# SilentView/EMCID

Measured on AMD Instinct MI355X. Metric: concept-edits/sec (1 000-concept batch, SD-v1.4), higher is better.
Workload: dtype f32 forward (2 x fp16 split MFMA, fp32 accumulate) + f64 solve

## Files before the change

### emcid_amd/csrc/clip_layers.hip

```cpp
#include "common.h"

#include <algorithm>

namespace emcid {

__global__ __launch_bounds__(256) void gather_rows16_kernel(const unsigned char* __restrict__ src, int64_t src_stride,
                                                             const int* __restrict__ idx, unsigned char* __restrict__ dst,
                                                             int64_t dst_stride, int row_bytes) {
    typedef unsigned int v4u __attribute__((ext_vector_type(4)));
    const int64_t r = blockIdx.x;
    const v4u* s = reinterpret_cast<const v4u*>(src + (int64_t)idx[r] * src_stride);
    v4u* d = reinterpret_cast<v4u*>(dst + r * dst_stride);
    for (int i = threadIdx.x; i < row_bytes / 16; i += 256) d[i] = s[i];
}

__global__ __launch_bounds__(256) void gather_f32_kernel(const float* __restrict__ src, const int* __restrict__ idx,
                                                          float* __restrict__ dst, int n) {
    const int i = blockIdx.x * 256 + threadIdx.x;
    if (i < n) dst[i] = src[idx[i]];
}

__device__ __forceinline__ unsigned long long fp_mix(unsigned long long x) {
    x ^= x >> 30; x *= 0xBF58476D1CE4E5B9ull; x ^= x >> 27; x *= 0x94D049BB133111EBull; x ^= x >> 31;
    return x;
// ... 37 lines not shown
        long long* e = table + 4 * b.slot[blockIdx.x];
        e[0] = (long long)reinterpret_cast<uintptr_t>(data); e[1] = bytes; e[2] = (long long)h; e[3] = 0;
    }
}

struct FpSkip { unsigned long long m[4]; };

__global__ __launch_bounds__(256) void fingerprint_check_kernel(const long long* table, long long first_slot, FpSkip skip, int* flag) {
    __shared__ unsigned long long lds[4];
    if ((skip.m[blockIdx.x >> 6] >> (blockIdx.x & 63)) & 1ull) return;
    const long long* e = table + 4 * (first_slot + blockIdx.x);
    const long long bytes = e[1];
    if (bytes <= 0) return;
    const unsigned long long h = fingerprint_of(reinterpret_cast<const unsigned char*>((uintptr_t)e[0]), bytes, lds);
    if (threadIdx.x == 0 && h != (unsigned long long)e[2]) atomicOr(flag, 1);
}

struct ClipWs {
    float* qkv;
    float* mid;
    uint32_t* ctx_p;
    float* ctx_s;
    uint32_t* z_p;
    float* z_s;
    float* f_scale;
    uint32_t* f_p;
    uint32_t* xq_p;
    float* xq_s;
    float* hs_q;
};

inline int64_t clip_ws_bytes(int64_t rows, int64_t h, int64_t d) {
    const int64_t r = round_up(rows, 64);
    return 4 * (r * 3 * h + r * h + r * h + r + r * h + r + 2 * r + r * d + r * h + r + r * h) + 16 * 16;
}

inline bool clip_ws_carve(void* base, int64_t bytes, int64_t rows, int64_t h, int64_t d, ClipWs& w) {
    if (base == nullptr || !aligned16(base) || bytes < clip_ws_bytes(rows, h, d)) return false;
    const int64_t r = round_up(rows, 64);
    char* p = (char*)base;
    auto take = [&](int64_t n4) { char* q = p; p += round_up(4 * n4, 16); return q; };
    w.qkv = (float*)take(r * 3 * h);
    w.mid = (float*)take(r * h);
    w.ctx_p = (uint32_t*)take(r * h);
    w.ctx_s = (float*)take(r);
    w.z_p = (uint32_t*)take(r * h);
    w.z_s = (float*)take(r);
    w.f_scale = (float*)take(2 * r);
    w.f_p = (uint32_t*)take(r * d);
    w.xq_p = (uint32_t*)take(r * h);
    w.xq_s = (float*)take(r);
    w.hs_q = (float*)take(r * h);
    return true;
}

}

using namespace emcid;

extern "C" {

int emcid_fingerprint_store(int64_t n, const void* const* data, const int64_t* bytes, const int64_t* slots, void* table,
                            int64_t table_slots, void* stream) {
    EMCID_CHECK_ARG(n >= 0 && table && (n == 0 || (data && bytes && slots)));
    for (int64_t i0 = 0; i0 < n; i0 += 32) {
        FpBatch b{};
        const int cnt = (int)std::min<int64_t>(32, n - i0);
        for (int i = 0; i < cnt; ++i) {
            EMCID_CHECK_ARG(data[i0 + i] && bytes[i0 + i] > 0 && bytes[i0 + i] % 16 == 0 && aligned16(data[i0 + i]) &&
                            slots[i0 + i] >= 0 && slots[i0 + i] < table_slots);
            b.data[i] = (const unsigned char*)data[i0 + i]; b.bytes[i] = bytes[i0 + i]; b.slot[i] = slots[i0 + i];
        }
        hipLaunchKernelGGL(fingerprint_store_kernel, dim3((unsigned)cnt), dim3(256), 0, (hipStream_t)stream, b, (long long*)table);
    }
    EMCID_CHECK_LAUNCH();
    return EMCID_OK;
}

int emcid_fingerprint_check(const void* table, int64_t table_slots, int64_t first_slot, int64_t n_slots, const uint64_t* skip_mask,
                            int* flag, void* stream) {
    EMCID_CHECK_ARG(table && flag && first_slot >= 0 && n_slots >= 0 && first_slot + n_slots <= table_slots && n_slots <= 256);
    if (n_slots == 0) return EMCID_OK;
    FpSkip skip{};
    if (skip_mask != nullptr)
        for (int w = 0; w < 4; ++w) skip.m[w] = skip_mask[w];
    hipLaunchKernelGGL(fingerprint_check_kernel, dim3((unsigned)n_slots), dim3(256), 0, (hipStream_t)stream, (const long long*)table,
                       (long long)first_slot, skip, flag);
    EMCID_CHECK_LAUNCH();
    return EMCID_OK;
}

int64_t emcid_clip_workspace_bytes(int64_t rows, int64_t h, int64_t d) { return clip_ws_bytes(rows, h, d); }

int emcid_clip_layer_head_sp16(const emcid_clip_layer_sp16* L, int64_t rows, int64_t h, int64_t d, int64_t heads, float attn_scale,
                               const int* anc, int64_t anc_ld, const int* depth, const int* rows_sel, int64_t n_sel,
                               const float* hs, const void* x_planes, const float* x_inv_scale, float* mid, void* f_planes,
                               float* f_scale, float* f_f32, void* workspace, int64_t workspace_bytes, void* stream) {
    EMCID_CHECK_ARG(L && rows > 0 && h > 0 && d > 0 && heads > 0 && h % heads == 0 && anc && depth && hs && x_planes && x_inv_scale);
    EMCID_CHECK_ARG(mid && f_planes && f_scale && n_sel > 0 && n_sel <= rows && (rows_sel != nullptr || n_sel == rows) && h % 32 == 0 && d % 32 == 0);
    ClipWs w;
    if (!clip_ws_carve(workspace, workspace_bytes, rows, h, d, w)) return fail(EMCID_ERR_BAD_ARG, __func__, "workspace too small or misaligned");
    hipStream_t st = (hipStream_t)stream;
    const int64_t D = h / heads;
    const float* q;
    int64_t ldq;
    const float* res;
    if (rows_sel == nullptr) {
        EMCID_TRY(emcid_linear_sp16_f32(x_planes, h, x_inv_scale, L->qkv_planes, h, L->qkv_inv_scale, L->qkv_bias, nullptr, 0, w.qkv,
                                        3 * h, nullptr, 0, nullptr, rows, 3 * h, h, 0, -1, stream));
        q = w.qkv, ldq = 3 * h, res = hs;
    } else {
        EMCID_TRY(emcid_linear_sp16_f32(x_planes, h, x_inv_scale, (const uint32_t*)L->qkv_planes + h * h, h, L->qkv_inv_scale + h,
                                        L->qkv_bias ? L->qkv_bias + h : nullptr, nullptr, 0, w.qkv + h, 3 * h, nullptr, 0, nullptr,
                                        rows, 2 * h, h, 0, -1, stream));
        {
            ScopedProf sp(KC_MISC, st);
            hipLaunchKernelGGL(gather_rows16_kernel, dim3((unsigned)n_sel), dim3(256), 0, st, (const unsigned char*)x_planes, 4 * h,
                               rows_sel, (unsigned char*)w.xq_p, 4 * h, (int)(4 * h));
            hipLaunchKernelGGL(gather_f32_kernel, dim3((unsigned)((n_sel + 255) / 256)), dim3(256), 0, st, x_inv_scale, rows_sel,
                               w.xq_s, (int)n_sel);
            hipLaunchKernelGGL(gather_rows16_kernel, dim3((unsigned)n_sel), dim3(256), 0, st, (const unsigned char*)hs, 4 * h,
                               rows_sel, (unsigned char*)w.hs_q, 4 * h, (int)(4 * h));
            EMCID_CHECK_LAUNCH();
        }
        EMCID_TRY(emcid_linear_sp16_f32(w.xq_p, h, w.xq_s, L->qkv_planes, h, L->qkv_inv_scale, L->qkv_bias, nullptr, 0, w.mid, h,
                                        nullptr, 0, nullptr, n_sel, h, h, 0, -1, stream));
        q = w.mid, ldq = h, res = w.hs_q;
    }
    EMCID_TRY(emcid_tree_attention_sp16(q, ldq, w.qkv + h, w.qkv + 2 * h, 3 * h, anc, anc_ld, depth, rows_sel, n_sel, heads, D,
                                        attn_scale, w.ctx_p, h, w.ctx_s, stream));
    EMCID_TRY(emcid_linear_sp16_f32(w.ctx_p, h, w.ctx_s, L->out_planes, h, L->out_inv_scale, L->out_bias, res, h, mid, h, nullptr,
                                    0, nullptr, n_sel, h, h, 0, -1, stream));
    EMCID_TRY(emcid_add_layernorm_sp16(mid, h, nullptr, 0, L->ln2_gamma, L->ln2_beta, L->ln2_eps, n_sel, h, nullptr, nullptr, w.z_p,
                                       h, w.z_s, L->fc1_bound, f_scale, stream));
    EMCID_TRY(emcid_linear_sp16_f32(w.z_p, h, w.z_s, L->fc1_planes, h, L->fc1_inv_scale, L->fc1_bias, nullptr, 0, f_f32, d,
                                    f_planes, d, f_scale, n_sel, d, h, L->act, -1, stream));
    return EMCID_OK;
}

int emcid_clip_layer_tail_sp16(const emcid_clip_layer_sp16* L, int64_t n, int64_t h, int64_t d, const void* f_planes,
                               const float* f_inv_scale, const float* mid, float* hs_out, const float* next_ln_gamma,
                               const float* next_ln_beta, float next_ln_eps, void* x_planes, float* x_inv_scale, void* stream) {
    EMCID_CHECK_ARG(L && n > 0 && h % 32 == 0 && d % 32 == 0 && f_planes && f_inv_scale && mid && hs_out);
    EMCID_TRY(emcid_linear_sp16_f32(f_planes, d, f_inv_scale, L->fc2_planes, d, L->fc2_inv_scale, L->fc2_bias, mid, h, hs_out, h,
                                    nullptr, 0, nullptr, n, h, d, 0, -1, stream));
    if (next_ln_gamma != nullptr) {
        EMCID_CHECK_ARG(next_ln_beta && x_planes && x_inv_scale);
        EMCID_TRY(emcid_add_layernorm_sp16(hs_out, h, nullptr, 0, next_ln_gamma, next_ln_beta, next_ln_eps, n, h, nullptr, nullptr,
                                           x_planes, h, x_inv_scale, nullptr, nullptr, stream));
    }
    return EMCID_OK;
}

int emcid_clip_edit_layer_tail_sp16(const emcid_clip_layer_sp16* L, int64_t n_rows, int64_t h, int64_t d, const float* f_f32,
                                    const void* f_planes, const float* f_inv_scale, const float* mid, const int64_t* lookup,
                                    const int64_t* seg, int64_t B, int64_t N, const float* zs_t, double edit_weight,
                                    int layers_left, double lam_ratio, const void* cov_factor_ws, int64_t n_layers,
                                    int64_t layer_index, int use_inverse, const float* W0, float* W, float* dW, float* K_out,
                                    float* Zc_out, void* k_planes, float* k_inv_scale, void* dual_ws, int64_t dual_ws_bytes,
                                    int* info_dev, void* linear_ws, int64_t linear_ws_bytes, float* hs_out,
                                    const float* next_ln_gamma, const float* next_ln_beta, float next_ln_eps, void* x_planes,
                                    float* x_inv_scale, void* stream) {
    EMCID_CHECK_ARG(L && n_rows > 0 && h % 32 == 0 && d % 32 == 0 && f_f32 && lookup && seg && B > 0 && N > 0 && zs_t);
    EMCID_CHECK_ARG(cov_factor_ws && W0 && W && K_out && Zc_out && dual_ws && info_dev && (hs_out == nullptr || (f_planes && f_inv_scale && mid)));
    EMCID_TRY(emcid_gather_mean_f32(f_f32, B, n_rows, d, 0, d, lookup, seg, N, K_out, d, stream));
    EMCID_CHECK_ARG((k_planes == nullptr) == (k_inv_scale == nullptr));
    if (k_planes != nullptr) {
        EMCID_TRY(emcid_split_rows_f16(K_out, d, N, d, k_planes, d, k_inv_scale, nullptr, stream));
        EMCID_TRY(emcid_linear_sp16_f32(k_planes, d, k_inv_scale, L->fc2_planes, d, L->fc2_inv_scale, L->fc2_bias, nullptr, 0, Zc_out, h,
                                        nullptr, 0, nullptr, N, h, d, 0, -1, stream));
    } else {
        EMCID_TRY(emcid_linear_ws_f32(K_out, d, W, d, L->fc2_bias, nullptr, 0, Zc_out, h, N, h, d, 0, -1, linear_ws, linear_ws_bytes, stream));
    }
    EMCID_TRY(emcid_edit_dual_apply_stage1_f64(K_out, Zc_out, zs_t, N, d, h, edit_weight, layers_left, lam_ratio, cov_factor_ws,
                                               n_layers, layer_index, 0, N, use_inverse, dual_ws, dual_ws_bytes, stream));
    EMCID_TRY(emcid_edit_dual_apply_stage2_f64(N, d, h, cov_factor_ws, n_layers, layer_index, use_inverse, 0, W0, W, dW, dual_ws,
                                               dual_ws_bytes, info_dev, stream));
    if (hs_out != nullptr) {
        EMCID_TRY(emcid_split_rows_f16(W, d, h, d, const_cast<void*>(L->fc2_planes), d, const_cast<float*>(L->fc2_inv_scale), nullptr,
                                       stream));
        EMCID_TRY(emcid_clip_layer_tail_sp16(L, n_rows, h, d, f_planes, f_inv_scale, mid, hs_out, next_ln_gamma, next_ln_beta,
                                             next_ln_eps, x_planes, x_inv_scale, stream));
    }
    return EMCID_OK;
}

int emcid_clip_layers_sp16(const emcid_clip_layer_sp16* layers, int64_t n_layers, int64_t rows, int64_t h, int64_t d, int64_t heads,
                           float attn_scale, const int* anc, int64_t anc_ld, const int* depth, float* hs, void* x_planes,
                           float* x_inv_scale, const float* next_ln_gamma, const float* next_ln_beta, float next_ln_eps,
                           void* workspace, int64_t workspace_bytes, void* stream) {
    EMCID_CHECK_ARG(layers && n_layers > 0 && hs && x_planes && x_inv_scale);
    ClipWs w;
    if (!clip_ws_carve(workspace, workspace_bytes, rows, h, d, w)) return fail(EMCID_ERR_BAD_ARG, __func__, "workspace too small or misaligned");
    for (int64_t i = 0; i < n_layers; ++i) {
        const emcid_clip_layer_sp16* L = layers + i;
        EMCID_TRY(emcid_clip_layer_head_sp16(L, rows, h, d, heads, attn_scale, anc, anc_ld, depth, nullptr, rows, hs, x_planes,
                                             x_inv_scale, w.mid, w.f_p, w.f_scale, nullptr, workspace, workspace_bytes, stream));
        const bool last = i + 1 == n_layers;
        const float* g = last ? next_ln_gamma : layers[i + 1].ln1_gamma;
        const float* b = last ? next_ln_beta : layers[i + 1].ln1_beta;
        const float eps = last ? next_ln_eps : layers[i + 1].ln1_eps;
        EMCID_TRY(emcid_clip_layer_tail_sp16(L, rows, h, d, w.f_p, w.f_scale + rows, w.mid, hs, g, b, eps, x_planes, x_inv_scale, stream));
    }
    return EMCID_OK;
}

}
```

### emcid_amd/csrc/edit_solve.hip

```cpp
#include "spd_solve.h"

namespace emcid {


__global__ __launch_bounds__(256) void prep_kr_kernel(const float* __restrict__ K, const float* __restrict__ Zc,
                                                       const float* __restrict__ zs_t, int N, int d, int h, double s,
                                                       double layers_left, double* __restrict__ Kt64, int Np, int dp,
                                                       double* __restrict__ Rt, int hp, double g = 1.0) {
    const int n = blockIdx.x;
    for (int j = threadIdx.x; j < dp; j += 256) {
        double v = 0.0;
        if (n < N && j < d) v = (double)K[(int64_t)n * d + j] * s * g;
        Kt64[(int64_t)n * dp + j] = v;
    }
    if (Rt) {
        for (int i = threadIdx.x; i < hp; i += 256) {
            double v = 0.0;
            if (n < N && i < h) {
                const float src = zs_t[(int64_t)n * h + i] - Zc[(int64_t)n * h + i];
                v = ((double)src * s) / layers_left * g;
            }
            Rt[(int64_t)n * hp + i] = v;
        }
    }
}

static void launch_prep_kr(const float* K, const float* Zc, const float* zs_t, int64_t N, int64_t d, int64_t h, double edit_weight,
                           int layers_left, double gain, double* Kt, int64_t Np, int64_t dp, double* R, int64_t hp, hipStream_t st) {
    ScopedProf sp(KC_PREP, st);
    hipLaunchKernelGGL(prep_kr_kernel, dim3((unsigned)Np), dim3(256), 0, st, K, Zc, zs_t, (int)N, (int)d, (int)h, sqrt(edit_weight / 0.5),
                       (double)layers_left, Kt, (int)Np, (int)dp, R, (int)hp, gain);
}

__global__ __launch_bounds__(256) void axpy_f32_kernel(float* __restrict__ W, const float* __restrict__ dW, int64_t n) {
    int64_t i = (int64_t)blockIdx.x * 256 + threadIdx.x;
    const int64_t stride = (int64_t)gridDim.x * 256;
    for (; i < n; i += stride) W[i] += dW[i];
}

__global__ __launch_bounds__(256) void apply_u_kernel(const double* __restrict__ U, const float* __restrict__ W0,
                                                       float* __restrict__ W, float* __restrict__ dW, int64_t n) {
    int64_t i = (int64_t)blockIdx.x * 256 + threadIdx.x;
    const int64_t stride = (int64_t)gridDim.x * 256;
    for (; i < n; i += stride) {
        const float f = (float)U[i];
        if (dW) dW[i] = f;
        if (W) W[i] = W0[i] + f;
    }
}

static int factor_and_solve(double* A, double* L, int64_t dp, int64_t lda, double* invw, int* info, double* B, double* Y,
                            int64_t rows, int64_t ldb, hipStream_t st) {
    return with_graph(make_key(GRAPH_FACTOR_SOLVE, {A, L, invw, info, B, Y}, {dp, lda, rows, ldb}), st, [&](hipStream_t s) {
        EMCID_TRY(cholesky_impl(A, L, dp, lda, invw, info, s));
        return cholesky_solve_impl(L, dp, lda, invw, B, Y, rows, ldb, s);
    });
}


struct CovPtrs { const float* c[32]; };
__global__ __launch_bounds__(256) void scale_cov_kernel(CovPtrs cov, int d, int dp, double lam, float cw, double* __restrict__ M,
                                                         int64_t s_mat) {
    const int l = blockIdx.y;
    const int i = blockIdx.x;
    const float* C = cov.c[l];
    double* row = M + l * s_mat + (int64_t)i * dp;
    for (int j = threadIdx.x; j <= i; j += 256) {
        double v;
        if (i < d) {
            const float c1 = C[(int64_t)i * d + j] * cw;
            v = lam * (double)(c1 / 0.5f);
        } else {
            v = (i == j) ? 1.0 : 0.0;
        }
        row[j] = v;
    }
}

static void assemble_dual_system(const double* P, const double* Q, int64_t dp, double* S, int Np, hipStream_t st,
                                 double* sk_work = nullptr) {
    ScopedProf sp(KC_ASSEMBLE, st);
    GemmShape g{P, dp, Q, dp, Np, Np, (int)dp, 1};
    if (Np >= 512 && sk_work && launch_gemm_f64_streamk2<true, true>(g, EpiAxpby{S, Np, 1.0, 0.0}, st, kStreamKWgs, sk_work, 1.0))
        return;
    hipLaunchKernelGGL(eye_f64_kernel, dim3((unsigned)Np), dim3(256), 0, st, S, Np);
    const int kt = (int)(dp / 16);
    g.ksplit = kt >= 64 ? 4 : kt >= 32 ? 2 : 1;
    launch_gemm_f64<true, true>(g, EpiAxpby{S, Np, 1.0, 1.0}, st, Np >= 512 ? 1 : 2);
}

__global__ __launch_bounds__(256) void transpose_f64_kernel(const double* __restrict__ src, int64_t lds_, double* __restrict__ dst,
                                                             int64_t ldd, int rows, int cols) {
    __shared__ double tile[32][33];
    const int bx = blockIdx.x * 32, by = blockIdx.y * 32;
    const int tx = threadIdx.x & 31, ty = threadIdx.x >> 5;
    for (int r = ty; r < 32; r += 8)
        tile[r][tx] = (by + r < rows && bx + tx < cols) ? src[(int64_t)(by + r) * lds_ + bx + tx] : 0.0;
    __syncthreads();
    for (int r = ty; r < 32; r += 8)
        if (bx + r < cols && by + tx < rows) dst[(int64_t)(bx + r) * ldd + by + tx] = tile[tx][r];
}

struct EditWorkspace {
    int64_t Np, dp, hp;
    int64_t off_A, off_L, off_inv, off_B, off_Y, off_R, total;
    EditWorkspace(int64_t N, int64_t d, int64_t h) {
        Np = round_up(N, NPAD);
        dp = round_up(d, NB);
        hp = round_up(h, 2);
        int64_t o = 0;
        off_A = o; o += dp * dp;
        off_L = o; o += dp * dp;
        off_inv = o; o += inv_doubles(dp);
        off_B = o; o += Np * dp;
        off_Y = o; o += Np * dp;
        off_R = o; o += Np * hp;
        total = o;
    }
};

int solve_schur_rhs(const double* R, int64_t hp, int64_t h, int64_t Np, const double* LS, const double* invS, const double* XT,
                    double* full_inv, double* RT, double* Y2, hipStream_t st) {
    hipLaunchKernelGGL(transpose_f64_kernel, dim3((unsigned)((hp + 31) / 32), (unsigned)(Np / 32)), dim3(256), 0, st, R, hp, RT, Np,
                       (int)Np, (int)hp);
    if (XT) {
        ScopedProf sp(KC_TRSM_DIAG, st);
        GemmShape f{RT, Np, XT, Np, (int)h, (int)Np, (int)Np, 0};
        f.tri = 1; f.pair = 1;
        launch_gemm_f64<true, false>(f, EpiAxpby{Y2, Np, 1.0, 0.0}, st);
        GemmShape b{Y2, Np, XT, Np, (int)h, (int)Np, (int)Np, 0};
        b.tri = 2; b.pair = 1;
        launch_gemm_f64<true, true>(b, EpiAxpby{RT, Np, 1.0, 0.0}, st);
    } else if (full_inv && Np <= 4096) {
        EMCID_TRY(build_full_inverse(LS, Np, Np, invS, full_inv, Y2, 1, 0, 0, st));
        ScopedProf sp(KC_TRSM_DIAG, st);
        GemmShape f{RT, Np, full_inv, Np, (int)h, (int)Np, (int)Np, 0};
        f.tri = 1; f.pair = 1;
        launch_gemm_f64<true, true>(f, EpiAxpby{Y2, Np, 1.0, 0.0}, st);
        GemmShape b{Y2, Np, full_inv, Np, (int)h, (int)Np, (int)Np, 0};
        b.tri = 2; b.pair = 1;
        launch_gemm_f64<true, false>(b, EpiAxpby{RT, Np, 1.0, 0.0}, st);
    } else {
        EMCID_TRY(cholesky_solve_impl(LS, Np, Np, invS, RT, Y2, h, Np, st));
    }
    return EMCID_OK;
}

}

using namespace emcid;

extern "C" {

int emcid_assemble_spd_f64(const float* C, int64_t ldc, const double* Kt64, int64_t Np, int64_t d, int64_t ldk, double lam,
                           float cw, double* A, int64_t lda, void* stream) {
    EMCID_CHECK_ARG(C && Kt64 && A && Np > 0 && d > 0);
    const int64_t dp = round_up(d, NB);
    EMCID_CHECK_ARG(lda >= dp && ldk >= dp && ldc >= d && (ldk % 2 == 0) && aligned16(Kt64));
    GemmShape p{Kt64, ldk, Kt64, ldk, (int)dp, (int)dp, (int)Np, 1};
    {
        ScopedProf sp(KC_ASSEMBLE, (hipStream_t)stream);
        launch_gemm_f64<false, false>(p, EpiAssemble{C, ldc, lam, cw, A, lda, (int)d}, (hipStream_t)stream);
    }
    EMCID_CHECK_LAUNCH();
    return EMCID_OK;
}

int emcid_delta_w_f64(const double* Rt, int64_t ldr, const double* Xt, int64_t ldx, int64_t Np, int64_t h, int64_t d,
                      const float* W0, float* W, int64_t ldw, float* dW, double* U, void* stream) {
    EMCID_CHECK_ARG(Rt && Xt && Np > 0 && h > 0 && d > 0 && ldr % 2 == 0 && ldx % 2 == 0 && aligned16(Rt) && aligned16(Xt));
    EMCID_CHECK_ARG((W == nullptr) || (W0 != nullptr));
    GemmShape p{Rt, ldr, Xt, ldx, (int)h, (int)d, (int)Np, 0};
    {
        ScopedProf sp(KC_DELTA_W, (hipStream_t)stream);
        launch_gemm_f64<false, false>(p, EpiDeltaW{W0, W, ldw, dW, d, U, d}, (hipStream_t)stream);
    }
    EMCID_CHECK_LAUNCH();
    return EMCID_OK;
}

int emcid_axpy_f32(float* W, const float* dW, int64_t n, void* stream) {
    EMCID_CHECK_ARG(W && dW && n > 0);
    int64_t blocks = (n + 255) / 256;
    if (blocks > 2048) blocks = 2048;
    hipLaunchKernelGGL(axpy_f32_kernel, dim3((unsigned)blocks), dim3(256), 0, (hipStream_t)stream, W, dW, n);
    EMCID_CHECK_LAUNCH();
    return EMCID_OK;
}

int64_t emcid_edit_workspace_bytes(int64_t N, int64_t d, int64_t h) {
    if (N <= 0 || d <= 0 || h <= 0) return 0;
    return EditWorkspace(N, d, h).total * (int64_t)sizeof(double);
}

static int edit_layer_impl(const float* K, const float* Zc, const float* zs_t, const float* C, int64_t N, int64_t d, int64_t h,
                           double lam, double edit_weight, int layers_left, int64_t n_lo, int64_t n_hi, const float* W0,
                           float* W, double* Xt_out, double* Rt_out, float* dW_out, double* U_out, void* workspace,
                           int64_t workspace_bytes, int* info_dev, void* stream) {
    EMCID_CHECK_ARG(K && Zc && zs_t && C && N > 0 && d > 0 && h > 0 && layers_left > 0 && workspace && info_dev);
    EMCID_CHECK_ARG(N < (1 << 24) && d <= 32768 && h <= 32768);
    EMCID_CHECK_ARG(0 <= n_lo && n_lo < n_hi && n_hi <= N);
    EMCID_CHECK_ARG((W == nullptr) || (W0 != nullptr));
    EMCID_CHECK_ARG(aligned16(workspace));
    EditWorkspace ws(N, d, h);
    EMCID_CHECK_WORKSPACE(workspace_bytes, ws.total * (int64_t)sizeof(double), " (see emcid_edit_workspace_bytes)");
    hipStream_t st = (hipStream_t)stream;
    double* base = (double*)workspace;
    double *A = base + ws.off_A, *L = base + ws.off_L, *inv = base + ws.off_inv;
    double *B = base + ws.off_B, *Y = base + ws.off_Y, *R = base + ws.off_R;
    const float cw = (float)(1.0 - edit_weight);
    const int64_t rows = n_hi - n_lo;

    launch_prep_kr(K, Zc, zs_t, N, d, h, edit_weight, layers_left, 1.0, B, ws.Np, ws.dp, R, ws.hp, st);
    EMCID_CHECK_LAUNCH();
    EMCID_TRY(emcid_assemble_spd_f64(C, d, B, ws.Np, d, ws.dp, lam, cw, A, ws.dp, stream));
    double* Bs = B + n_lo * ws.dp;
    EMCID_TRY(factor_and_solve(A, L, ws.dp, ws.dp, inv, info_dev, Bs, Y + n_lo * ws.dp, rows, ws.dp, st));
    if (W || dW_out || U_out)
        EMCID_TRY(emcid_delta_w_f64(R + n_lo * ws.hp, ws.hp, Bs, ws.dp, rows, h, d, W0, W, d, dW_out, U_out, stream));
    if (Xt_out)
        hipLaunchKernelGGL(copy2d_f64_kernel, dim3((unsigned)rows), dim3(256), 0, st, Bs, ws.dp, Xt_out, d, (int)rows, (int)d);
    if (Rt_out)
        hipLaunchKernelGGL(copy2d_f64_kernel, dim3((unsigned)rows), dim3(256), 0, st, R + n_lo * ws.hp, ws.hp, Rt_out, h,
                           (int)rows, (int)h);
    EMCID_CHECK_LAUNCH();
    return EMCID_OK;
}

int emcid_edit_layer_f64(const float* K, const float* Zc, const float* zs_t, const float* C, int64_t N, int64_t d, int64_t h,
                         double lam, double edit_weight, int layers_left, const float* W0, float* W, double* Xt_out,
                         double* Rt_out, float* dW_out, void* workspace, int64_t workspace_bytes, int* info_dev,
                         void* stream) {
    return edit_layer_impl(K, Zc, zs_t, C, N, d, h, lam, edit_weight, layers_left, 0, N, W0, W, Xt_out, Rt_out, dW_out,
                           nullptr, workspace, workspace_bytes, info_dev, stream);
}

int emcid_edit_layer_shard_f64(const float* K, const float* Zc, const float* zs_t, const float* C, int64_t N, int64_t d,
                               int64_t h, double lam, double edit_weight, int layers_left, int64_t n_lo, int64_t n_hi,
                               double* U_partial, double* Xt_out, double* Rt_out, void* workspace, int64_t workspace_bytes,
                               int* info_dev, void* stream) {
    EMCID_CHECK_ARG(U_partial != nullptr);
    return edit_layer_impl(K, Zc, zs_t, C, N, d, h, lam, edit_weight, layers_left, n_lo, n_hi, nullptr, nullptr, Xt_out,
                           Rt_out, nullptr, U_partial, workspace, workspace_bytes, info_dev, stream);
}

int emcid_apply_update_f32(const double* U, const float* W0, float* W, float* dW, int64_t n, void* stream) {
    EMCID_CHECK_ARG(U && n > 0 && (W || dW) && ((W == nullptr) || (W0 != nullptr)));
    int64_t blocks = (n + 255) / 256;
    if (blocks > 2048) blocks = 2048;
    hipLaunchKernelGGL(apply_u_kernel, dim3((unsigned)blocks), dim3(256), 0, (hipStream_t)stream, U, W0, W, dW, n);
    EMCID_CHECK_LAUNCH();
    return EMCID_OK;
}


int64_t emcid_cov_factor_workspace_bytes(int64_t n_layers, int64_t d) {
    if (n_layers <= 0 || d <= 0) return 0;
    return CovFactorLayout(n_layers, d).total * (int64_t)sizeof(double);
}

int emcid_factor_cov_f64(const float* const* C_host_list, int64_t n_layers, int64_t d, double lam, double edit_weight,
                         void* workspace, int64_t workspace_bytes, int* info_dev, void* stream) {
    EMCID_CHECK_ARG(C_host_list && n_layers > 0 && n_layers <= 32 && d > 0 && d <= 32768 && workspace && info_dev);
    EMCID_CHECK_ARG(aligned16(workspace));
    const CovFactorLayout cov(n_layers, d);
    EMCID_CHECK_WORKSPACE(workspace_bytes, cov.total * (int64_t)sizeof(double), " (see emcid_cov_factor_workspace_bytes)");
    const int64_t dp = cov.dp, s_mat = cov.s_mat, s_inv = cov.s_inv;
    double *Mb = cov.M(workspace, 0), *Lb = cov.L(workspace, 0), *Ib = cov.I(workspace, 0);
    CovPtrs cp;
    for (int i = 0; i < 32; ++i) cp.c[i] = i < n_layers ? C_host_list[i] : nullptr;
    for (int i = 0; i < n_layers; ++i) EMCID_CHECK_ARG(cp.c[i] != nullptr);
    const float cw = (float)(1.0 - edit_weight);
    hipStream_t st = (hipStream_t)stream;
    GraphKey key = make_key(GRAPH_FACTOR_COV, {Mb, info_dev}, {n_layers, d, 0, 0, 0});
    memcpy(&key.num[2], &lam, sizeof(double));
    memcpy(&key.num[3], &cw, sizeof(float));
    for (int i = 0; i < n_layers; ++i)
        if (i < 6) key.ptr[2 + i] = cp.c[i]; else key.num[4] = key.num[4] * 1000003 + (int64_t)(uintptr_t)cp.c[i];
    return with_graph(key, st, [&](hipStream_t s) {
        hipLaunchKernelGGL(scale_cov_kernel, dim3((unsigned)dp, (unsigned)n_layers), dim3(256), 0, s, cp, (int)d, (int)dp, lam, cw,
                           Mb, s_mat);
        return cholesky_serial(Mb, Lb, dp, dp, Ib, info_dev, s, (int)n_layers, s_mat, s_inv);
    });
}

int emcid_cov_inverse_f64(void* cov_factor_ws, int64_t n_layers, int64_t d, int64_t first_layer, int64_t count, void* stream) {
    EMCID_CHECK_ARG(cov_factor_ws && n_layers > 0 && n_layers <= 32 && d > 0 && d <= 32768 && aligned16(cov_factor_ws));
    EMCID_CHECK_ARG(0 <= first_layer && count > 0 && first_layer + count <= n_layers);
    const CovFactorLayout cov(n_layers, d);
    const int64_t dp = cov.dp;
    double* Mb = cov.M(cov_factor_ws, first_layer);
    const double *Lb = cov.L(cov_factor_ws, first_layer), *Ib = cov.I(cov_factor_ws, first_layer);
    double* Xb = cov.X(cov_factor_ws, first_layer);
    return with_graph(make_key(GRAPH_COV_INVERSE, {Mb, Lb, Ib, Xb}, {dp, count}), (hipStream_t)stream, [&](hipStream_t s) {
        return build_full_inverse(Lb, dp, dp, Ib, Xb, Mb, (int)count, cov.s_mat, cov.s_inv, s);
    });
}

__global__ __launch_bounds__(256) void cov_factor_rescale_kernel(const double* src, double* dst, int64_t off_L, int64_t off_I,
                                                                 int64_t off_X, int64_t s_mat, int64_t s_inv, int dp, int n_tri,
                                                                 double gain_L, double gain_inv, int with_inverse) {
    const int64_t layer = blockIdx.y;
    const int region = blockIdx.z;
    if (region == 1) {
        const double2* s = reinterpret_cast<const double2*>(src + off_I + layer * s_inv);
        double2* o = reinterpret_cast<double2*>(dst + off_I + layer * s_inv);
        for (int64_t i = (int64_t)blockIdx.x * 256 + threadIdx.x; i < s_inv / 2; i += (int64_t)gridDim.x * 256) {
            double2 v = s[i];
            v.x *= gain_inv;
            v.y *= gain_inv;
            o[i] = v;
        }
        return;
    }
    if (region == 2 && !with_inverse) return;
    const int t = blockIdx.x;
    if (t >= n_tri) return;
    int I = (int)((sqrtf(8.0f * (float)t + 1.0f) - 1.0f) * 0.5f);
    while ((I + 1) * (I + 2) / 2 <= t) ++I;
    while (I * (I + 1) / 2 > t) --I;
    const int J = t - I * (I + 1) / 2;
    const int64_t base = (region == 0 ? off_L : off_X) + layer * s_mat + (int64_t)I * NB * dp + (int64_t)J * NB;
    const double g = region == 0 ? gain_L : gain_inv;
    for (int e = threadIdx.x; e < NB * (NB / 2); e += 256) {
        const int r = e / (NB / 2), c2 = e % (NB / 2);
        const int64_t at = base + (int64_t)r * dp + 2 * c2;
        double2 v = *reinterpret_cast<const double2*>(src + at);
        v.x *= g;
        v.y *= g;
        *reinterpret_cast<double2*>(dst + at) = v;
    }
}

int emcid_cov_factor_rescale_f64(const void* src_ws, void* dst_ws, int64_t workspace_bytes, int64_t n_layers, int64_t d, double a,
                                 int with_inverse, void* stream) {
    EMCID_CHECK_ARG(src_ws && dst_ws && n_layers > 0 && n_layers <= 32 && d > 0 && d <= 32768);
    EMCID_CHECK_ARG(aligned16(src_ws) && aligned16(dst_ws) && a > 0.0 && a < 1e300);
    const CovFactorLayout cov(n_layers, d);
    EMCID_CHECK_WORKSPACE(workspace_bytes, cov.total * (int64_t)sizeof(double), " (see emcid_cov_factor_workspace_bytes)");
    const int64_t dp = cov.dp, s_inv = cov.s_inv, nt = dp / NB;
    EMCID_CHECK_ARG(s_inv % 2 == 0);
    const double* src = (const double*)src_ws;
    const int n_tri = (int)(nt * (nt + 1) / 2);
    const double root = sqrt(a);
    hipLaunchKernelGGL(cov_factor_rescale_kernel, dim3((unsigned)n_tri, (unsigned)n_layers, 3), dim3(256), 0, (hipStream_t)stream,
                       src, (double*)dst_ws, (int64_t)(cov.L(src, 0) - src), (int64_t)(cov.I(src, 0) - src), (int64_t)(cov.X(src, 0) - src),
                       cov.s_mat, s_inv, (int)dp, n_tri, root, 1.0 / root, with_inverse);
    EMCID_CHECK_LAUNCH();
    return EMCID_OK;
}

static double* dual_block(void* workspace, int64_t N, int64_t d, int64_t h, int64_t DualWorkspace::*off) {
    if (!workspace || N <= 0 || d <= 0 || h <= 0) return nullptr;
    return (double*)workspace + DualWorkspace(N, d, h).*off;
}

int64_t emcid_edit_dual_workspace_bytes(int64_t N, int64_t d, int64_t h) {
    if (N <= 0 || d <= 0 || h <= 0) return 0;
    return DualWorkspace(N, d, h).total * (int64_t)sizeof(double);
}

#define EMCID_CHECK_DUAL_STAGE1_ARGS()                                                                            \
    EMCID_CHECK_ARG(K && Zc && zs_t && N > 0 && d > 0 && h > 0 && layers_left > 0 && cov_factor_ws && workspace); \
    EMCID_CHECK_ARG(0 <= layer_index && layer_index < n_layers && 0 <= n_lo && n_lo < n_hi && n_hi <= N);         \
    EMCID_CHECK_ARG(lam_ratio > 0.0 && lam_ratio < 1e300)

int emcid_edit_dual_stage1_f64(const float* K, const float* Zc, const float* zs_t, int64_t N, int64_t d, int64_t h,
                               double edit_weight, int layers_left, double lam_ratio, const void* cov_factor_ws, int64_t n_layers,
                               int64_t layer_index, int64_t n_lo, int64_t n_hi, int use_inverse, void* workspace,
                               int64_t workspace_bytes, void* stream) {
    EMCID_CHECK_DUAL_STAGE1_ARGS();
    DualWorkspace ws(N, d, h);
    EMCID_CHECK_WORKSPACE(workspace_bytes, ws.total * (int64_t)sizeof(double), "");
    hipStream_t st = (hipStream_t)stream;
    double* base = (double*)workspace;
    double *Kt = base + ws.off_K, *Pt = base + ws.off_P, *Y = base + ws.off_Y, *R = base + ws.off_R;
    const int64_t dp = ws.dp;
    const CovFactorLayout cov(n_layers, d);
    const double *Lb = cov.L(cov_factor_ws, layer_index), *Ib = cov.I(cov_factor_ws, layer_index);
    launch_prep_kr(K, Zc, zs_t, N, d, h, edit_weight, layers_left, 1.0 / sqrt(lam_ratio), Kt, ws.Np, dp, R, ws.hp, st);
    const int64_t rows = n_hi - n_lo;
    if (use_inverse) {
        const double* Xb = cov.X(cov_factor_ws, layer_index);
        apply_inverse_forward(Xb, dp, Kt + n_lo * dp, Y + n_lo * dp, (int)rows, st, base + ws.off_SK);
        apply_inverse_backward(Xb, dp, Y + n_lo * dp, (int)rows, (int)dp, Pt + n_lo * dp, dp, st, base + ws.off_SK);
        EMCID_CHECK_LAUNCH();
        return EMCID_OK;
    }
    if (hipMemcpyAsync(Pt + n_lo * dp, Kt + n_lo * dp, rows * dp * sizeof(double), hipMemcpyDeviceToDevice, st) != hipSuccess)
        return fail(EMCID_ERR_HIP, __func__, "hipMemcpyAsync");
    return with_graph(make_key(GRAPH_DUAL_STAGE1, {Lb, Ib, Pt + n_lo * dp, Y + n_lo * dp}, {dp, rows}), st, [&](hipStream_t q) {
        return cholesky_solve_impl(Lb, dp, dp, Ib, Pt + n_lo * dp, Y + n_lo * dp, rows, dp, q);
    });
}

double* emcid_edit_dual_pt(void* workspace, int64_t N, int64_t d, int64_t h) { return dual_block(workspace, N, d, h, &DualWorkspace::off_P); }

int emcid_edit_dual_stage2_f64(int64_t N, int64_t d, int64_t h, double lam_ratio, const float* W0, float* W, double* adjk_out, double* Rt_out,
                               float* dW_out, void* workspace, int64_t workspace_bytes, int* info_dev, void* stream) {
    EMCID_CHECK_ARG(N > 0 && d > 0 && h > 0 && workspace && info_dev && ((W == nullptr) || (W0 != nullptr)));
    EMCID_CHECK_ARG(lam_ratio > 0.0 && lam_ratio < 1e300);
    DualWorkspace ws(N, d, h);
    EMCID_CHECK_WORKSPACE(workspace_bytes, ws.total * (int64_t)sizeof(double), "");
    hipStream_t st = (hipStream_t)stream;
    double* base = (double*)workspace;
    double *Kt = base + ws.off_K, *Pt = base + ws.off_P, *R = base + ws.off_R, *S = base + ws.off_S, *LS = base + ws.off_LS;
    double *invS = base + ws.off_invS, *PT = base + ws.off_PT, *Y2 = base + ws.off_Y2;
    const int64_t dp = ws.dp, Np = ws.Np;
    EMCID_TRY(with_graph(make_key(GRAPH_DUAL_STAGE2,{Kt, Pt, S, LS, invS, PT, Y2, info_dev}, {dp, Np, N}), st, [&](hipStream_t q) {
        if (Np > N)
            hipLaunchKernelGGL(zero_f64_kernel, dim3(256), dim3(256), 0, q, Pt + N * dp, (Np - N) * dp);
        assemble_dual_system(Pt, Kt, dp, S, (int)Np, q, base + ws.off_SK);
        EMCID_TRY(cholesky_impl(S, LS, Np, Np, invS, info_dev, q));
        hipLaunchKernelGGL(transpose_f64_kernel, dim3((unsigned)(dp / 32), (unsigned)(Np / 32)), dim3(256), 0, q, Pt, dp, PT, Np,
                           (int)Np, (int)dp);
        return cholesky_solve_impl(LS, Np, Np, invS, PT, Y2, dp, Np, q);
    }));
    if (W || dW_out) {
        ScopedProf sp(KC_DELTA_W, st);
        GemmShape g{R, ws.hp, PT, Np, (int)h, (int)d, (int)Np, 0};
        launch_gemm_f64<false, true>(g, EpiDeltaW{W0, W, d, dW_out, d, nullptr, d}, st);
    }
    const double root = sqrt(lam_ratio);
    if (adjk_out)
        hipLaunchKernelGGL(copy2d_f64_kernel, dim3((unsigned)d), dim3(256), 0, st, PT, Np, adjk_out, N, (int)d, (int)N, 1.0 / root);
    if (Rt_out) hipLaunchKernelGGL(copy2d_f64_kernel, dim3((unsigned)N), dim3(256), 0, st, R, ws.hp, Rt_out, h, (int)N, (int)h, root);
    EMCID_CHECK_LAUNCH();
    return EMCID_OK;
}

int emcid_edit_dual_apply_stage1_f64(const float* K, const float* Zc, const float* zs_t, int64_t N, int64_t d, int64_t h,
                                     double edit_weight, int layers_left, double lam_ratio, const void* cov_factor_ws, int64_t n_layers,
                                     int64_t layer_index, int64_t n_lo, int64_t n_hi, int use_inverse, void* workspace,
                                     int64_t workspace_bytes, void* stream) {
    EMCID_CHECK_DUAL_STAGE1_ARGS();
    DualWorkspace ws(N, d, h);
    EMCID_CHECK_WORKSPACE(workspace_bytes, ws.total * (int64_t)sizeof(double), "");
    hipStream_t st = (hipStream_t)stream;
    double* base = (double*)workspace;
    double *Kt = base + ws.off_K, *Bs = base + ws.off_P, *Yt = base + ws.off_Y, *R = base + ws.off_R;
    const int64_t dp = ws.dp;
    const CovFactorLayout cov(n_layers, d);
    const double *Lb = cov.L(cov_factor_ws, layer_index), *Ib = cov.I(cov_factor_ws, layer_index);
    launch_prep_kr(K, Zc, zs_t, N, d, h, edit_weight, layers_left, 1.0 / sqrt(lam_ratio), Kt, ws.Np, dp, R, ws.hp, st);
    const int64_t rows = n_hi - n_lo;
    if (use_inverse) {
        const int64_t gemm_rows = (n_lo == 0 && n_hi == N) ? ws.Np : rows;
        apply_inverse_forward(cov.X(cov_factor_ws, layer_index), dp, Kt + n_lo * dp, Yt + n_lo * dp, (int)gemm_rows, st,
                              base + ws.off_SK);
        if (gemm_rows != ws.Np && ws.Np > N)
            hipLaunchKernelGGL(zero_f64_kernel, dim3(256), dim3(256), 0, st, Yt + N * dp, (ws.Np - N) * dp);
        EMCID_CHECK_LAUNCH();
        return EMCID_OK;
    }
    if (ws.Np > N) hipLaunchKernelGGL(zero_f64_kernel, dim3(256), dim3(256), 0, st, Yt + N * dp, (ws.Np - N) * dp);
    if (hipMemcpyAsync(Bs + n_lo * dp, Kt + n_lo * dp, rows * dp * sizeof(double), hipMemcpyDeviceToDevice, st) != hipSuccess)
        return fail(EMCID_ERR_HIP, __func__, "hipMemcpyAsync");
    return with_graph(make_key(GRAPH_APPLY_STAGE1,{Lb, Ib, Bs + n_lo * dp, Yt + n_lo * dp}, {dp, rows}), st, [&](hipStream_t q) {
        trsm_forward(Lb, dp, dp, OB, Ib, Bs + n_lo * dp, dp, Yt + n_lo * dp, dp, (int)rows, q);
        return check_launch("emcid_edit_dual_apply_stage1_f64");
    });
}

double* emcid_edit_dual_yt(void* workspace, int64_t N, int64_t d, int64_t h) { return dual_block(workspace, N, d, h, &DualWorkspace::off_Y); }

int emcid_edit_dual_apply_assemble_f64(int64_t N, int64_t d, int64_t h, void* workspace, int64_t workspace_bytes, void* stream) {
    EMCID_CHECK_ARG(N > 0 && d > 0 && h > 0 && workspace);
    DualWorkspace ws(N, d, h);
    EMCID_CHECK_WORKSPACE(workspace_bytes, ws.total * (int64_t)sizeof(double), "");
    hipStream_t st = (hipStream_t)stream;
    double* base = (double*)workspace;
    double *Yt = base + ws.off_Y, *S = base + ws.off_S;
    const int64_t dp = ws.dp, Np = ws.Np;
    assemble_dual_system(Yt, Yt, dp, S, (int)Np, st, base + ws.off_SK);
    EMCID_CHECK_LAUNCH();
    return EMCID_OK;
}

int emcid_edit_dual_apply_stage2_f64(int64_t N, int64_t d, int64_t h, const void* cov_factor_ws, int64_t n_layers,
                                     int64_t layer_index, int use_inverse, int assembled, const float* W0, float* W,
                                     float* dW_out, void* workspace, int64_t workspace_bytes, int* info_dev, void* stream) {
    EMCID_CHECK_ARG(N > 0 && d > 0 && h > 0 && workspace && info_dev && cov_factor_ws && ((W == nullptr) || (W0 != nullptr)));
    EMCID_CHECK_ARG(0 <= layer_index && layer_index < n_layers && (W || dW_out));
    DualWorkspace ws(N, d, h);
    EMCID_CHECK_WORKSPACE(workspace_bytes, ws.total * (int64_t)sizeof(double), "");
    hipStream_t st = (hipStream_t)stream;
    double* base = (double*)workspace;
    double *Yt = base + ws.off_Y, *R = base + ws.off_R, *S = base + ws.off_S, *LS = base + ws.off_LS, *invS = base + ws.off_invS;
    double *RT = base + ws.off_PT, *Y2 = base + ws.off_Y2, *V = base + ws.off_V, *U = base + ws.off_U;
    const int64_t dp = ws.dp, Np = ws.Np, hp = ws.hp;
    const CovFactorLayout cov(n_layers, d);
    const double *Lb = cov.L(cov_factor_ws, layer_index), *Ib = cov.I(cov_factor_ws, layer_index);
    static const int shadow_env = env_flag("EMCID_SHADOW_P", 1);
    bool shadow = shadow_env && use_inverse && cholesky_takes_shadow(Np);
    if (shadow && shadow_env == 1) {
        const int64_t ntl = (dp + SH_BN - 1) / SH_BN, nb = Np / NB;
        const int64_t steps = ((ntl + 1) * (SH_BN / 16) + nb - 1) / nb;
        const int64_t wgs = ((Np + SH_BM - 1) / SH_BM) * ((ntl + 1) / 2), rounds = (wgs + 239) / 240;
        shadow = rounds * (9.0 + 1.5 * (double)steps) <= 50.0;
    }
    double* P = base + ws.off_P;
    const double* X = use_inverse ? cov.X(cov_factor_ws, layer_index) : nullptr;
    const bool p_first = !shadow && use_inverse && Np < h;
    const bool xrow = cholesky_takes_shadow(Np);
    double *XT = base + ws.off_XT, *TT = base + ws.off_TT;
    EMCID_TRY(with_graph(make_key(GRAPH_APPLY_STAGE2, {Yt, R, S, LS, RT, V, U, info_dev},
                                  {dp, Np, N, hp, (int64_t)(uintptr_t)Lb,
                                   use_inverse + 2 * (assembled != 0) + 4 * (int)shadow + 8 * h + ((int64_t)p_first << 31) + ((int64_t)xrow << 30) + (d << 32)}),
                         st,
                         [&](hipStream_t q) {
        if (!assembled) {
            assemble_dual_system(Yt, Yt, dp, S, (int)Np, q, base + ws.off_SK);
        }
        if (p_first) apply_inverse_backward(X, dp, Yt, (int)Np, (int)dp, P, dp, q, base + ws.off_SK);
        ShadowJob job{Yt, dp, X, dp, P, dp, (int)Np, (int)dp, (int)dp, 0, nullptr, 0, 0, 0};
        job.wgs = (int)((Np + SH_BM - 1) / SH_BM) * (int)(((dp + SH_BN - 1) / SH_BN + 1) / 2);
        const XrowJob xj{XT, Np, TT};
        EMCID_TRY(cholesky_impl(S, LS, Np, Np, invS, info_dev, q, shadow ? &job : nullptr, xrow ? &xj : nullptr));
        EMCID_TRY(solve_schur_rhs(R, hp, h, Np, LS, invS, xrow ? XT : nullptr, S, RT, Y2, q));
        if (!shadow && !p_first) {
            ScopedProf sp(KC_DELTA_W, q);
            GemmShape g{RT, Np, Yt, dp, (int)h, (int)dp, (int)Np, 0};
            launch_gemm_f64<true, false>(g, EpiAxpby{V, dp, 1.0, 0.0}, q);
        }
        if (!use_inverse) trsm_backward(Lb, dp, dp, OB, Ib, V, dp, U, dp, (int)h, q);
        return check_launch("emcid_edit_dual_apply_stage2_f64");
    }));
    if (shadow || p_first) {
        ScopedProf sp(KC_DELTA_W, st);
        GemmShape g{RT, Np, P, dp, (int)h, (int)d, (int)Np, 0};
        launch_gemm_f64<true, false>(g, EpiDeltaW{W0, W, d, dW_out, d, nullptr, 0}, st, -1);
        EMCID_CHECK_LAUNCH();
        return EMCID_OK;
    }
    if (use_inverse)
        apply_inverse_backward(X, dp, V, (int)h, (int)dp, U, dp, st, base + ws.off_SK);
    hipLaunchKernelGGL(apply_u2d_kernel, dim3((unsigned)h), dim3(256), 0, st, U, dp, W0, W, dW_out, (int)d);
    EMCID_CHECK_LAUNCH();
    return EMCID_OK;
}

__global__ __launch_bounds__(256) void add_identity_f64_kernel(double* __restrict__ S, int n) {
    const int i = blockIdx.x * 256 + threadIdx.x;
    if (i < n) S[(int64_t)i * n + i] += 1.0;
}

static int check_tiles(const int* tiles, int n_tiles, int64_t dp) {
    if (!tiles || n_tiles <= 0 || n_tiles > 256) return 0;
    for (int i = 0; i < n_tiles; ++i)
        if (tiles[i] < 0 || (int64_t)tiles[i] * NB >= dp || (i > 0 && tiles[i] <= tiles[i - 1])) return 0;
    return 1;
}

int emcid_edit_dual_cols_stage1_f64(const float* K, const float* Zc, const float* zs_t, int64_t N, int64_t d, int64_t h,
                                    double edit_weight, int layers_left, double lam_ratio, const void* cov_factor_ws, int64_t n_layers,
                                    int64_t layer_index, const int* tiles_host, int n_tiles, void* workspace,
                                    int64_t workspace_bytes, void* stream) {
    EMCID_CHECK_ARG(K && Zc && zs_t && N > 0 && d > 0 && h > 0 && layers_left > 0 && cov_factor_ws && workspace);
    EMCID_CHECK_ARG(0 <= layer_index && layer_index < n_layers && lam_ratio > 0.0 && lam_ratio < 1e300);
    DualWorkspace ws(N, d, h);
    EMCID_CHECK_ARG(check_tiles(tiles_host, n_tiles, ws.dp));
    EMCID_CHECK_WORKSPACE(workspace_bytes, ws.total * (int64_t)sizeof(double), "");
    hipStream_t st = (hipStream_t)stream;
    double* base = (double*)workspace;
    double *Kt = base + ws.off_K, *Yc = base + ws.off_Y, *R = base + ws.off_R, *S = base + ws.off_S, *sk = base + ws.off_SK;
    const int64_t dp = ws.dp, Np = ws.Np;
    const double* X = CovFactorLayout(n_layers, d).X(cov_factor_ws, layer_index);
    launch_prep_kr(K, Zc, zs_t, N, d, h, edit_weight, layers_left, 1.0 / sqrt(lam_ratio), Kt, Np, dp, R, ws.hp, st);
    for (int i = 0; i < n_tiles; ++i) {
        const int64_t t = tiles_host[i], kd = (t + 1) * NB;
        ScopedProf sp(KC_INV_APPLY, st);
        GemmShape g{Kt, dp, X + t * NB * dp, dp, (int)Np, NB, (int)kd, 0};
        if (!launch_gemm_f64_streamk2<true, true>(g, EpiAxpby{Yc + (int64_t)i * NB, dp, 1.0, 0.0}, st, kStreamKWgs, sk))
            return fail(EMCID_ERR_BAD_ARG, __func__, "more output tiles than stream-K ticket counters");
    }
    {
        ScopedProf sp(KC_ASSEMBLE, st);
        GemmShape g{Yc, dp, Yc, dp, (int)Np, (int)Np, n_tiles * NB, 1};
        if (!launch_gemm_f64_streamk2<true, true>(g, EpiAxpby{S, Np, 1.0, 0.0}, st, kStreamKWgs, sk, 0.0))
            return fail(EMCID_ERR_BAD_ARG, __func__, "more output tiles than stream-K ticket counters");
    }
    EMCID_CHECK_LAUNCH();
    return EMCID_OK;
}

double* emcid_edit_dual_s(void* workspace, int64_t N, int64_t d, int64_t h) { return dual_block(workspace, N, d, h, &DualWorkspace::off_S); }

double* emcid_edit_dual_u(void* workspace, int64_t N, int64_t d, int64_t h) { return dual_block(workspace, N, d, h, &DualWorkspace::off_U); }

int emcid_edit_dual_cols_stage2_f64(int64_t N, int64_t d, int64_t h, const void* cov_factor_ws, int64_t n_layers,
                                    int64_t layer_index, const int* tiles_host, int n_tiles, void* workspace,
                                    int64_t workspace_bytes, int* info_dev, void* stream) {
    EMCID_CHECK_ARG(N > 0 && d > 0 && h > 0 && workspace && info_dev && cov_factor_ws);
    EMCID_CHECK_ARG(0 <= layer_index && layer_index < n_layers);
    DualWorkspace ws(N, d, h);
    EMCID_CHECK_ARG(check_tiles(tiles_host, n_tiles, ws.dp));
    EMCID_CHECK_WORKSPACE(workspace_bytes, ws.total * (int64_t)sizeof(double), "");
    hipStream_t st = (hipStream_t)stream;
    double* base = (double*)workspace;
    double *Yc = base + ws.off_Y, *R = base + ws.off_R, *S = base + ws.off_S, *LS = base + ws.off_LS, *invS = base + ws.off_invS;
    double *RT = base + ws.off_PT, *Y2 = base + ws.off_Y2, *V = base + ws.off_V, *U = base + ws.off_U;
    const int64_t dp = ws.dp, Np = ws.Np, hp = ws.hp;
    const double* X = CovFactorLayout(n_layers, d).X(cov_factor_ws, layer_index);
    const int w = n_tiles * NB;
    const bool xrow = cholesky_takes_shadow(Np);
    EMCID_TRY(with_graph(make_key(GRAPH_COLS_STAGE2,{Yc, R, S, LS, RT, V, U, info_dev}, {dp, Np, N, hp, (int64_t)w + ((int64_t)xrow << 40)}), st, [&](hipStream_t q) {
        hipLaunchKernelGGL(add_identity_f64_kernel, dim3((unsigned)((Np + 255) / 256)), dim3(256), 0, q, S, (int)Np);
        const XrowJob xj{base + ws.off_XT, Np, base + ws.off_TT};
        EMCID_TRY(cholesky_impl(S, LS, Np, Np, invS, info_dev, q, nullptr, xrow ? &xj : nullptr));
        EMCID_TRY(solve_schur_rhs(R, hp, h, Np, LS, invS, xrow ? xj.Xt : nullptr, nullptr, RT, Y2, q));
        {
            ScopedProf sp(KC_DELTA_W, q);
            GemmShape g{RT, Np, Yc, dp, (int)h, w, (int)Np, 0};
            launch_gemm_f64<true, false>(g, EpiAxpby{V, dp, 1.0, 0.0}, q);
        }
        hipLaunchKernelGGL(zero2d_f64_kernel, dim3((unsigned)h, 1u), dim3(256), 0, q, U, dp, (int64_t)0, (int)dp);
        return check_launch("emcid_edit_dual_cols_stage2_f64");
    }));
    for (int i = 0; i < n_tiles; ++i) {
        const int64_t t = tiles_host[i], kd = (t + 1) * NB;
        ScopedProf sp(KC_INV_APPLY, st);
        GemmShape g{V + (int64_t)i * NB, dp, X + t * NB * dp, dp, (int)h, (int)kd, NB, 0};
        launch_gemm_f64<true, false>(g, EpiAxpby{U, dp, 1.0, 1.0}, st);
    }
    EMCID_CHECK_LAUNCH();
    return EMCID_OK;
}

int emcid_apply_update2d_f32(const double* U, int64_t ldu, const float* W0, float* W, float* dW, int64_t h, int64_t d, void* stream) {
    EMCID_CHECK_ARG(U && h > 0 && d > 0 && ldu >= d && (W || dW) && ((W == nullptr) || (W0 != nullptr)));
    hipLaunchKernelGGL(apply_u2d_kernel, dim3((unsigned)h), dim3(256), 0, (hipStream_t)stream, U, ldu, W0, W, dW, (int)d);
    EMCID_CHECK_LAUNCH();
    return EMCID_OK;
}

}
```

### emcid_amd/csrc/gemm_sp16.hip

```cpp
#include "common.h"
#include "sp16.h"

#include <algorithm>

namespace emcid {

typedef _Float16 v8h __attribute__((ext_vector_type(8)));
typedef _Float16 v4h __attribute__((ext_vector_type(4)));
typedef float v16f __attribute__((ext_vector_type(16)));
typedef float v4f __attribute__((ext_vector_type(4)));
typedef unsigned int v4u __attribute__((ext_vector_type(4)));

#ifndef SP16_ONE_SLOT
#define SP16_ONE_SLOT 0
#endif
constexpr int SPK = 32;

enum SpAct : int { SP_ACT_NONE = 0, SP_ACT_QUICK_GELU = 1, SP_ACT_GELU_ERF = 2 };

template <int V> struct SpIC { static constexpr int value = V; };

__device__ __forceinline__ bool sp_al16(const void* p) { return (reinterpret_cast<uintptr_t>(p) & 15) == 0; }

struct SpArgs {
// ... 538 lines not shown
            __builtin_amdgcn_sched_barrier(0);
            if (DBG != 1 && DBG != 3 && it + 2 < T) issue(it + 2, cur);
            if (DBG != 3 && it + 1 < T) fread(oth, SpIC<S ^ 1>{});
            __builtin_amdgcn_sched_barrier(0);
            mfmas(sc);
            __builtin_amdgcn_sched_barrier(0);
            __builtin_amdgcn_s_waitcnt(0xc07f);
            __builtin_amdgcn_sched_barrier(0);
        };
        auto body_full = [&](int it, auto sc) __attribute__((always_inline)) {
            constexpr int S = decltype(sc)::value;
            constexpr int NREAD = 2 * (MJ + NI), NMFMA = 3 * MJ * NI, MPG = (2 * MJ * NI) / NREAD < 1 ? 1 : (2 * MJ * NI) / NREAD;
            static_assert(NMFMA >= PXW + PWW + MPG * NREAD, "MFMAs to hide the issue under");
            constexpr int NDMA = PXW + PWW;
            unsigned char* cur = smem + (it & 1) * STAGE;
            unsigned char* oth = smem + ((it + 1) & 1) * STAGE;
            __builtin_amdgcn_s_waitcnt(0x0f70);
            __builtin_amdgcn_s_barrier();
            __builtin_amdgcn_sched_barrier(0);
            if (DBG != 1 && DBG != 3) issue(it + 2, cur);
            if (DBG != 3) fread(oth, SpIC<S ^ 1>{});
            mfmas(sc);
#pragma unroll
            for (int g = 0; g < NDMA; ++g) {
                __builtin_amdgcn_sched_group_barrier(0x008, 1, 0);
                __builtin_amdgcn_sched_group_barrier(0x020, 1, 0);
            }
#pragma unroll
            for (int g = 0; g < NREAD; ++g) {
                __builtin_amdgcn_sched_group_barrier(0x008, MPG, 0);
                __builtin_amdgcn_sched_group_barrier(0x100, 1, 0);
            }
            __builtin_amdgcn_sched_group_barrier(0x008, NMFMA - NDMA - MPG * NREAD, 0);
            __builtin_amdgcn_sched_barrier(0);
            __builtin_amdgcn_s_waitcnt(0xc07f);
            __builtin_amdgcn_sched_barrier(0);
        };
        int it = 0;
        if constexpr (ILV) {
            for (; it + 3 < T; it += 2) {
                body_full(it, SpIC<0>{});
                body_full(it + 1, SpIC<1>{});
            }
        }
        for (; it + 1 < T; it += 2) {
            body(it, SpIC<0>{});
            body(it + 1, SpIC<1>{});
        }
        if (it < T) body(it, SpIC<0>{});
    } else {
        for (int it = 0; it < T; ++it) {
            unsigned char* cur = smem + (it & 1) * STAGE;
            unsigned char* oth = smem + ((it + 1) & 1) * STAGE;
            const bool more = DBG != 3 && it + 1 < T;
#pragma unroll
            for (int j = 0; j < MJ / 2; ++j)
#pragma unroll
                for (int i = 0; i < NI; ++i) mfma3(i, j, SpIC<0>{});
            __builtin_amdgcn_sched_barrier(0);
            __builtin_amdgcn_s_waitcnt(0x0070);
            __builtin_amdgcn_s_barrier();
            __builtin_amdgcn_sched_barrier(0);
            if (DBG != 1 && DBG != 3 && it + 2 < T) issue(it + 2, cur);
            if (more) {
#pragma unroll
                for (int j = 0; j < MJ / 2; ++j) fread_x(oth, j, SpIC<0>{});
            }
            __builtin_amdgcn_sched_barrier(0);
#pragma unroll
            for (int j = MJ / 2; j < MJ - 1; ++j) {
#pragma unroll
                for (int i = 0; i < NI; ++i) mfma3(i, j, SpIC<0>{});
                __builtin_amdgcn_sched_barrier(0);
                if (more) fread_x(oth, j, SpIC<0>{});
                __builtin_amdgcn_sched_barrier(0);
            }
#pragma unroll
            for (int i = 0; i < NI; ++i) {
                mfma3(i, MJ - 1, SpIC<0>{});
                __builtin_amdgcn_sched_barrier(0);
                if (more) fread_w(oth, i, SpIC<0>{});
                __builtin_amdgcn_sched_barrier(0);
            }
            if (more) fread_x(oth, MJ - 1, SpIC<0>{});
            __builtin_amdgcn_sched_barrier(0);
        }
    }
}

template <int BM, int BN, int NT>
struct SpSidePre {
    static constexpr int NSV = (BM + BN + NT - 1) / NT;
    const SpArgs& a;
    int m0, n0;
    float* side;
    float sv0[NSV], sv1[NSV];
    __device__ __forceinline__ void load() {
        const int tid = threadIdx.x;
#pragma unroll
        for (int q = 0; q < NSV; ++q) {
            const int e = tid + q * NT;
            sv0[q] = sv1[q] = 0.f;
            if (e < BM) {
                sv0[q] = a.xs[min(m0 + e, a.M - 1)];
                sv1[q] = a.ps != nullptr ? a.ps[min(m0 + e, a.M - 1)] : 1.f;
            } else if (e < BM + BN) {
                sv0[q] = a.ws[min(n0 + e - BM, a.N - 1)];
                sv1[q] = a.bias != nullptr ? a.bias[min(n0 + e - BM, a.N - 1)] : 0.f;
            }
        }
    }
    __device__ __forceinline__ void store() {
        const int tid = threadIdx.x;
#pragma unroll
        for (int q = 0; q < NSV; ++q) {
            const int e = tid + q * NT;
            if (e < BM) side[e] = sv0[q], side[BM + e] = sv1[q];
            else if (e < BM + BN) side[2 * BM + e - BM] = sv0[q], side[2 * BM + BN + e - BM] = sv1[q];
        }
    }
};

template <int MJ, int NI, int WM, int WN, int NSLOT, int DBG, int WPE = 2, bool ILV = (NSLOT == 2)>
__global__ __launch_bounds__(64 * WM * WN) __attribute__((amdgpu_waves_per_eu(WPE, WPE))) void linear_sp16_dma16_kernel(SpArgs a) {
    constexpr int NWV = WM * WN, BM = 16 * MJ * WM, BN = 16 * NI * WN;
    constexpr int STAGE = (BM + BN) * 128;
    static_assert(2 * STAGE >= NWV * 2048 * NI, "the epilogue's LDS regions");
    constexpr int SIDE = 4 * (2 * BM + 2 * BN);
    __shared__ __attribute__((aligned(1024))) unsigned char smem[2 * STAGE + SIDE];
    const int per = (a.tiles + 7) / 8;
    const int tile = (blockIdx.x & 7) * per + (blockIdx.x >> 3);
    if (tile >= a.tiles || (int)(blockIdx.x >> 3) >= per) return;
    int bm, bn;
    sp_tile_of(a, tile, bm, bn);
    long long t_begin = 0;
    if constexpr (DBG == 2) t_begin = (long long)__builtin_amdgcn_s_memrealtime();
    const int m0 = bm * BM, n0 = bn * BN;
    v4f acc[NI][MJ];
    long long clk[2] = {0, 0};
    SpSidePre<BM, BN, 64 * NWV> pre{a, m0, n0, reinterpret_cast<float*>(smem + 2 * STAGE)};
    sp_accumulate16<MJ, NI, WM, WN, NSLOT, DBG, ILV>(a.X + (int64_t)m0 * a.ldx, a.ldx, a.M - m0, a.W + (int64_t)n0 * a.ldw, a.ldw, a.N - n0,
                                                     a.K / SPK, smem, acc, pre, clk);
    if constexpr (DBG == 2) {
        const long long e_clk = (long long)__builtin_amdgcn_s_memtime(), e_real = (long long)__builtin_amdgcn_s_memrealtime();
        if (a.stamps != nullptr && threadIdx.x == 0) {
            long long* st = a.stamps + 8 * (int64_t)blockIdx.x;
            st[0] = clk[0]; st[1] = e_clk; st[2] = clk[1]; st[3] = e_real; st[4] = t_begin;
        }
    }
    sp_finish16<MJ, NI, WM, WN>(a, m0, n0, smem, reinterpret_cast<const float*>(smem + 2 * STAGE), acc);
    if constexpr (DBG == 2) {
        if (a.stamps != nullptr && threadIdx.x == 0) a.stamps[8 * (int64_t)blockIdx.x + 5] = (long long)__builtin_amdgcn_s_memrealtime();
    }
}

__device__ __forceinline__ void sp_split8(const v4f& a, const v4f& b, float s, v4u& hi, v4u& lo) {
    v8h h, l;
#pragma unroll
    for (int e = 0; e < 8; ++e) {
        const float t = (e < 4 ? a[e] : b[e - 4]) * s;
        h[e] = (_Float16)t;
        l[e] = (_Float16)(t - (float)h[e]);
    }
    hi = *reinterpret_cast<v4u*>(&h);
    lo = *reinterpret_cast<v4u*>(&l);
}

__global__ __launch_bounds__(256) void split_rows_kernel(const float* __restrict__ X, int64_t ldx, int rows, int K,
                                                          uint32_t* __restrict__ P, int64_t ldp, float* __restrict__ inv_scale,
                                                          float* __restrict__ max_row_norm) {
    const int lane = threadIdx.x & 63;
    const int64_t row = (int64_t)blockIdx.x * 4 + (threadIdx.x >> 6);
    if (row >= rows) return;
    const float* x = X + row * ldx;
    const int ng = K / 8;
    float amax = 0.f, ss = 0.f;
    for (int g = lane; g < ng; g += 64) {
        const v4f a = *reinterpret_cast<const v4f*>(x + 8 * g), b = *reinterpret_cast<const v4f*>(x + 8 * g + 4);
#pragma unroll
        for (int e = 0; e < 4; ++e) {
            amax = fmaxf(amax, fmaxf(fabsf(a[e]), fabsf(b[e])));
            ss += a[e] * a[e] + b[e] * b[e];
        }
    }
#pragma unroll
    for (int o = 32; o > 0; o >>= 1) {
        amax = fmaxf(amax, __shfl_xor(amax, o, 64));
        ss += __shfl_xor(ss, o, 64);
    }
    if (max_row_norm != nullptr && lane == 0)
        atomicMax(reinterpret_cast<unsigned int*>(max_row_norm), __float_as_uint(sqrtf(ss) * 1.0001f));
    float s, inv;
    sp_scale_of(amax, s, inv);
    if (lane == 0) inv_scale[row] = inv;
    uint32_t* p = P + row * ldp;
    for (int g = lane; g < ng; g += 64) {
        const v4f a = *reinterpret_cast<const v4f*>(x + 8 * g), b = *reinterpret_cast<const v4f*>(x + 8 * g + 4);
        v4u hi, lo;
        sp_split8(a, b, s, hi, lo);
        *reinterpret_cast<v4u*>(p + 8 * g) = hi;
        *reinterpret_cast<v4u*>(p + 8 * g + 4) = lo;
    }
}

__global__ __launch_bounds__(256) void gram_colmax_kernel(const float* __restrict__ X, int64_t ldx, const float* __restrict__ rw, int t,
                                                           int d, int rows_per_wg, unsigned* __restrict__ cmax) {
    const int c4 = blockIdx.x * 256 + threadIdx.x;
    if (4 * c4 >= d) return;
    const int r0 = blockIdx.y * rows_per_wg, r1 = min(t, r0 + rows_per_wg);
    v4f m = {0.f, 0.f, 0.f, 0.f};
    int r = r0;
    for (; r + 8 <= r1; r += 8) {
        v4f x[8];
        float w[8];
#pragma unroll
        for (int u = 0; u < 8; ++u) {
            x[u] = *reinterpret_cast<const v4f*>(X + (int64_t)(r + u) * ldx + 4 * c4);
            w[u] = rw != nullptr ? rw[r + u] : 1.f;
        }
#pragma unroll
        for (int u = 0; u < 8; ++u)
#pragma unroll
            for (int e = 0; e < 4; ++e) m[e] = fmaxf(m[e], fabsf(x[u][e] * w[u]));
    }
    for (; r < r1; ++r) {
        const v4f x = *reinterpret_cast<const v4f*>(X + (int64_t)r * ldx + 4 * c4);
        const float w = rw != nullptr ? rw[r] : 1.f;
#pragma unroll
        for (int e = 0; e < 4; ++e) m[e] = fmaxf(m[e], fabsf(x[e] * w));
    }
#pragma unroll
    for (int e = 0; e < 4; ++e) atomicMax(cmax + 4 * c4 + e, __float_as_uint(m[e]));
}

__global__ __launch_bounds__(256) void gram_transpose_split_kernel(const float* __restrict__ X, int64_t ldx, const float* __restrict__ rw,
                                                                    int t, int d, const unsigned* __restrict__ cmax,
                                                                    uint32_t* __restrict__ P, int64_t ldp, float* __restrict__ inv_scale) {
    __shared__ float tile[64][65];
    const int t0 = blockIdx.x * 64, d0 = blockIdx.y * 64, tid = threadIdx.x;
    for (int v = tid; v < 64 * 16; v += 256) {
        const int r = v >> 4, c = (v & 15) * 4;
        v4f x = {0.f, 0.f, 0.f, 0.f};
        float w = 1.f;
        if (t0 + r < t && d0 + c < d) {
            x = *reinterpret_cast<const v4f*>(X + (int64_t)(t0 + r) * ldx + d0 + c);
            if (rw != nullptr) w = rw[t0 + r];
        }
#pragma unroll
        for (int e = 0; e < 4; ++e) tile[r][c + e] = x[e] * w;
    }
    __syncthreads();
#pragma unroll
    for (int u = 0; u < 2; ++u) {
        const int w = tid + 256 * u, f = w >> 3, g = w & 7;
        if (d0 + f >= d) continue;
        float s, inv;
        sp_scale_of(__uint_as_float(cmax[d0 + f]), s, inv);
        if (blockIdx.x == 0 && g == 0) inv_scale[d0 + f] = inv;
        v4f a, b;
#pragma unroll
        for (int e = 0; e < 4; ++e) a[e] = tile[8 * g + e][f], b[e] = tile[8 * g + 4 + e][f];
        v4u hi, lo;
        sp_split8(a, b, s, hi, lo);
        uint32_t* dst = P + (int64_t)(d0 + f) * ldp + t0 + 8 * g;
        *reinterpret_cast<v4u*>(dst) = hi;
        *reinterpret_cast<v4u*>(dst + 4) = lo;
    }
}

struct GramSpArgs {
    const uint32_t* XT; int64_t ld; const float* inv; float* G; int64_t ldg; int d, K, tiles_side, ks;
};

__global__ __launch_bounds__(256) __attribute__((amdgpu_waves_per_eu(2, 2))) void gram_sp16_kernel(GramSpArgs g) {
    constexpr int MJ = 4, NI = 4, WM = 2, WN = 2, BT = 128;
    __shared__ __attribute__((aligned(1024))) unsigned char smem[2 * (2 * BT) * 128];
    const int n_lower = g.tiles_side * (g.tiles_side + 1) / 2, items = n_lower * g.ks, per = (items + 7) / 8;
    const int item = (blockIdx.x & 7) * per + (blockIdx.x >> 3);
    if (item >= items || (int)(blockIdx.x >> 3) >= per) return;
    const int tile = item / g.ks, part = item - tile * g.ks;
    int bm = (int)((sqrtf(8.f * (float)tile + 1.f) - 1.f) * 0.5f);
    while (bm * (bm + 1) / 2 > tile) --bm;
    while ((bm + 1) * (bm + 2) / 2 <= tile) ++bm;
    const int bn = tile - bm * (bm + 1) / 2;
    const int T = g.K / SPK, it_lo = (int)((int64_t)part * T / g.ks), it_hi = (int)((int64_t)(part + 1) * T / g.ks);
    if (it_hi <= it_lo) return;
    const int c0 = bn * BT, r0 = bm * BT;
    const uint32_t* base = g.XT + (int64_t)it_lo * SPK;
    v4f acc[NI][MJ];
    long long clk[2];
    SpNoPre pre;
    sp_accumulate16<MJ, NI, WM, WN, 2, 0, true>(base + (int64_t)c0 * g.ld, g.ld, g.d - c0, base + (int64_t)r0 * g.ld, g.ld, g.d - r0,
                                                it_hi - it_lo, smem, acc, pre, clk);
    const int tid = threadIdx.x, lane = tid & 63, wave = tid >> 6, l15 = lane & 15, l4 = lane >> 4;
    const int wm0 = (wave / WN) * (16 * MJ), wn0 = (wave % WN) * (16 * NI);
    float rinv[NI][4];
#pragma unroll
    for (int i = 0; i < NI; ++i)
#pragma unroll
        for (int e = 0; e < 4; ++e) rinv[i][e] = g.inv[min(r0 + wn0 + 16 * i + 4 * l4 + e, g.d - 1)];
#pragma unroll
    for (int j = 0; j < MJ; ++j) {
        const int col = c0 + wm0 + 16 * j + l15;
        const float sc = g.inv[min(col, g.d - 1)];
#pragma unroll
        for (int i = 0; i < NI; ++i)
#pragma unroll
            for (int e = 0; e < 4; ++e) {
                const int row = r0 + wn0 + 16 * i + 4 * l4 + e;
                if (row < g.d && col < g.d) unsafeAtomicAdd(g.G + (int64_t)row * g.ldg + col, acc[i][j][e] * (sc * rinv[i][e]));
            }
    }
}

struct SpCfg { int bm, bn; };
static const SpCfg kSpCfgs[] = {{128, 128}, {80, 128}, {64, 64}, {160, 128}, {64, 64}};
inline long long* g_sp16_stamps = nullptr;

// ... 123 lines not shown
```

### emcid_amd/csrc/sp16.h

```cpp
#pragma once
#include <hip/hip_runtime.h>
#include <stdint.h>

namespace emcid {

typedef _Float16 sp_v4h __attribute__((ext_vector_type(4)));

__device__ __forceinline__ void sp_scale_of(float amax, float& s, float& inv) {
    int ex = (int)((__float_as_uint(amax) >> 23) & 0xff);
    ex = ex == 0 ? 1 : (ex == 255 ? 254 : ex);
    int e = 141 - ex;
    e = e > 120 ? 120 : (e < -120 ? -120 : e);
    s = __uint_as_float((unsigned)(e + 127) << 23);
    inv = __uint_as_float((unsigned)(127 - e) << 23);
}

__device__ __forceinline__ void sp_store4(uint32_t* row_planes, int col, float x0, float x1, float x2, float x3, float s) {
    sp_v4h h, l;
    const float t0 = x0 * s, t1 = x1 * s, t2 = x2 * s, t3 = x3 * s;
    h[0] = (_Float16)t0; h[1] = (_Float16)t1; h[2] = (_Float16)t2; h[3] = (_Float16)t3;
    l[0] = (_Float16)(t0 - (float)h[0]); l[1] = (_Float16)(t1 - (float)h[1]);
    l[2] = (_Float16)(t2 - (float)h[2]); l[3] = (_Float16)(t3 - (float)h[3]);
    unsigned char* dst = reinterpret_cast<unsigned char*>(row_planes) + (col >> 3) * 32 + ((col >> 2) & 1) * 8;
    *reinterpret_cast<sp_v4h*>(dst) = h;
    *reinterpret_cast<sp_v4h*>(dst + 16) = l;
}

}
```

### emcid_amd/csrc/spd_solve.h

```cpp
#pragma once
#include "common.h"
#include "gemm_f64.h"

namespace emcid {


#define EMCID_GEMM_F64_INSTANCES(X)                                                                        \
    X void launch_gemm_f64<true, false, EpiAxpby>(GemmShape, EpiAxpby, hipStream_t, int);                     \
    X void launch_gemm_f64<true, true, EpiAxpby>(GemmShape, EpiAxpby, hipStream_t, int);                      \
    X bool launch_gemm_f64_streamk2<true, true>(GemmShape, EpiAxpby, hipStream_t, int, double*, double);      \
    X bool launch_gemm_f64_streamk2<true, false>(GemmShape, EpiAxpby, hipStream_t, int, double*, double);     \
    X void launch_gemm_f64<false, true, EpiAxpby>(GemmShape, EpiAxpby, hipStream_t, int);                     \
    X void launch_gemm_f64<false, false, EpiAxpby>(GemmShape, EpiAxpby, hipStream_t, int);                    \
    X void launch_gemm_f64<false, false, EpiAssemble>(GemmShape, EpiAssemble, hipStream_t, int);              \
    X void launch_gemm_f64<false, false, EpiDeltaW>(GemmShape, EpiDeltaW, hipStream_t, int);                  \
    X void launch_gemm_f64<false, true, EpiDeltaW>(GemmShape, EpiDeltaW, hipStream_t, int);                   \
    X void launch_gemm_f64<true, false, EpiDeltaW>(GemmShape, EpiDeltaW, hipStream_t, int);
EMCID_GEMM_F64_INSTANCES(extern template)

struct ShadowJob {
    const double* A; int64_t lda;
    const double* B; int64_t ldb;
    double* C; int64_t ldc;
    int M, N, K;
    int wgs;
    long long* stamps;
    int xcd_gx;
    int nofast;
    int fuse_pair;
};

struct XrowJob {
    double* Xt; int64_t ldx;
    double* Tt;
};
constexpr int SH_BM = 64, SH_BN = 128;

inline bool cholesky_takes_shadow(int64_t dp) {
    return dp <= 2048 && dp >= 2 * NB;
}
int cholesky_serial(double* A, double* L, int64_t dp, int64_t lda, double* invw, int* info, hipStream_t st, int nbatch = 1,
                    int64_t s_mat = 0, int64_t s_inv = 0);
int cholesky_impl(double* A, double* L, int64_t dp, int64_t lda, double* invw, int* info, hipStream_t st,
                  const ShadowJob* shadow = nullptr, const XrowJob* xrow = nullptr);
void trsm_forward(const double* L, int64_t ldl, int64_t n, int blk, const double* inv, double* B, int64_t ldb, double* Out,
                  int64_t ldo, int rows, hipStream_t st);
void trsm_backward(const double* L, int64_t ldl, int64_t n, int blk, const double* inv, double* B, int64_t ldb, double* Out,
                   int64_t ldo, int rows, hipStream_t st);
int cholesky_solve_impl(const double* L, int64_t dp, int64_t lda, const double* invw, double* Bt, double* Yt, int64_t Mrows,
                        int64_t ldb, hipStream_t st);
int build_full_inverse(const double* L, int64_t dp, int64_t lda, const double* invw, double* X, double* T, int nbatch,
                       int64_t s_mat, int64_t s_inv, hipStream_t st);
constexpr int kStreamKWgs = 256;
void apply_inverse_forward(const double* X, int64_t dp, const double* Kt, double* Yt, int rows, hipStream_t st,
                           double* sk_work = nullptr);
void apply_inverse_backward(const double* X, int64_t dp, const double* V, int rows, int ncols, double* C, int64_t ldc,
                            hipStream_t st, double* sk_work = nullptr);
void assemble_schur_system(const double* Yk, int64_t ldy, int64_t dp, const double* Lkp, int64_t ldl, int64_t M, double* S, int N,
                           int Np, hipStream_t st);


struct CovFactorLayout {
    int64_t n_layers, dp, s_mat, s_inv, total;
    CovFactorLayout(int64_t n_layers_, int64_t d)
        : n_layers(n_layers_), dp(round_up(d, NB)), s_mat(dp * dp), s_inv(inv_doubles(dp)), total(n_layers * (3 * s_mat + s_inv)) {}
    double* M(const void* ws, int64_t l) const { return (double*)ws + l * s_mat; }
    double* L(const void* ws, int64_t l) const { return (double*)ws + n_layers * s_mat + l * s_mat; }
    double* I(const void* ws, int64_t l) const { return (double*)ws + 2 * n_layers * s_mat + l * s_inv; }
    double* X(const void* ws, int64_t l) const { return (double*)ws + n_layers * (2 * s_mat + s_inv) + l * s_mat; }
};

struct DualWorkspace {
    int64_t Np, dp, hp;
    int64_t off_K, off_P, off_Y, off_R, off_S, off_LS, off_invS, off_PT, off_Y2, off_V, off_U, off_SK, off_XT, off_TT, total;
    DualWorkspace(int64_t N, int64_t d, int64_t h) {
        Np = round_up(N, NB);
        dp = round_up(d, NB);
        hp = round_up(h, 2);
        int64_t o = 0;
        off_K = o; o += Np * dp;
        off_P = o; o += Np * dp;
        off_Y = o; o += Np * dp;
        off_R = o; o += Np * hp;
        off_S = o; o += Np * Np;
        off_LS = o; o += Np * Np;
        off_invS = o; o += inv_doubles(Np);
        off_PT = o; o += dp * Np;
        off_Y2 = o; o += dp * Np;
        off_V = o; o += hp * dp;
        off_U = o; o += hp * dp;
        off_SK = o; o += streamk_workspace_doubles(kStreamKWgs);
        off_XT = o; o += Np * Np;
        off_TT = o; o += Np * NB;
        total = o;
    }
};

int solve_schur_rhs(const double* R, int64_t hp, int64_t h, int64_t Np, const double* LS, const double* invS, const double* XT,
                    double* full_inv, double* RT, double* Y2, hipStream_t st);


static __global__ __launch_bounds__(256) void copy2d_f64_kernel(const double* __restrict__ src, int64_t lds_, double* __restrict__ dst,
                                                                 int64_t ldd, int rows, int cols, double scale = 1.0) {
    const int r = blockIdx.x;
    for (int c = threadIdx.x; c < cols; c += 256) dst[(int64_t)r * ldd + c] = src[(int64_t)r * lds_ + c] * scale;
}

static __global__ __launch_bounds__(256) void zero_f64_kernel(double* __restrict__ p, int64_t n) {
    int64_t i = (int64_t)blockIdx.x * 256 + threadIdx.x;
    const int64_t stride = (int64_t)gridDim.x * 256;
    for (; i < n; i += stride) p[i] = 0.0;
}

static __global__ __launch_bounds__(256) void zero2d_f64_kernel(double* __restrict__ p, int64_t ld, int64_t s_batch, int cols) {
    double* row = p + blockIdx.y * s_batch + (int64_t)blockIdx.x * ld;
    for (int j = threadIdx.x; j < cols; j += 256) row[j] = 0.0;
}

static __global__ __launch_bounds__(256) void eye_f64_kernel(double* __restrict__ S, int n) {
    const int i = blockIdx.x;
    for (int j = threadIdx.x; j < n; j += 256) S[(int64_t)i * n + j] = (i == j) ? 1.0 : 0.0;
}

static __global__ __launch_bounds__(256) void apply_u2d_kernel(const double* __restrict__ U, int64_t ldu, const float* __restrict__ W0,
                                                                float* __restrict__ W, float* __restrict__ dW, int d) {
    const int i = blockIdx.x;
    for (int j = threadIdx.x; j < d; j += 256) {
        const float f = (float)U[(int64_t)i * ldu + j];
        if (dW) dW[(int64_t)i * d + j] = f;
        if (W) W[(int64_t)i * d + j] = W0[(int64_t)i * d + j] + f;
    }
}

}
```

### emcid_amd/hip.py

```python
from __future__ import annotations

import ctypes as C
import math
import os
import threading
from pathlib import Path
from typing import Optional

import torch

_LIB_PATH = Path(__file__).resolve().parent / "csrc" / "libemcid_hip.so"
_lib = None

EXPORTS = [
    "emcid_abi_version", "emcid_last_error", "emcid_gram_accumulate_f32", "emcid_symmetrize_lower_f32",
    "emcid_gather_mean_f32", "emcid_edit_workspace_bytes", "emcid_edit_layer_f64", "emcid_assemble_spd_f64",
    "emcid_cholesky_f64", "emcid_cholesky_solve_f64", "emcid_delta_w_f64", "emcid_dgemm_f64", "emcid_dgemm_ex_f64", "emcid_dgemm_batched_f64", "emcid_streamk_workspace_bytes", "emcid_dgemm_streamk_f64", "emcid_debug_streamk_stamps", "emcid_debug_step_stamps", "emcid_debug_linear_sp16_stamps", "emcid_fingerprint_store", "emcid_fingerprint_check", "emcid_axpy_f32",
    "emcid_profile_enable", "emcid_profile_collect", "emcid_attention_f32", "emcid_edit_layer_shard_f64",
    "emcid_apply_update_f32", "emcid_inverse_workspace_doubles", "emcid_quick_gelu_f32", "emcid_add_layernorm_f32", "emcid_embed_layernorm_f32", "emcid_tree_attention_f32", "emcid_debug_leaf_stamps",
    "emcid_cov_factor_workspace_bytes", "emcid_factor_cov_f64", "emcid_cov_inverse_f64", "emcid_cov_factor_rescale_f64",
    "emcid_edit_dual_workspace_bytes",
    "emcid_edit_dual_stage1_f64", "emcid_edit_dual_pt", "emcid_edit_dual_stage2_f64",
    "emcid_edit_dual_apply_stage1_f64", "emcid_edit_dual_yt", "emcid_edit_dual_apply_stage2_f64",
    "emcid_edit_dual_apply_assemble_f64",
    "emcid_edit_dual_preserve_workspace_bytes", "emcid_edit_layer_dual_preserve_f64",
    "emcid_session_retain_workspace_bytes", "emcid_session_retain_f64", "emcid_session_step_norms_f64",
    "emcid_session_release_workspace_bytes", "emcid_session_release_f64",
    "emcid_cov_factor_fold_workspace_bytes", "emcid_cov_factor_fold_f64",
    "emcid_edit_lu_workspace_bytes", "emcid_edit_layer_lu_f64", "emcid_lu_solve_f64",
    "emcid_edit_dual_cols_stage1_f64", "emcid_edit_dual_s", "emcid_edit_dual_u", "emcid_edit_dual_cols_stage2_f64",
    "emcid_apply_update2d_f32", "emcid_linear_f32", "emcid_linear_ws_f32", "emcid_linear_workspace_bytes",
    "emcid_split_rows_f16", "emcid_linear_sp16_f32", "emcid_gram_sp16_workspace_bytes", "emcid_gram_sp16_workspace_bytes_for", "emcid_gram_accumulate_sp16_f32", "emcid_add_layernorm_sp16", "emcid_embed_layernorm_sp16",
    "emcid_tree_attention_sp16", "emcid_tree_attention_sp16_supported", "emcid_clip_workspace_bytes",
    "emcid_clip_layer_head_sp16", "emcid_clip_layer_tail_sp16", "emcid_clip_layers_sp16", "emcid_clip_edit_layer_tail_sp16",
]
PROF_CLASSES = ["prep", "assemble", "chol_leaf", "chol_panel", "chol_trail", "trsm_diag", "trsm_update", "delta_w",
                "gram", "gather", "dgemm", "misc", "inv_build", "chol_inner", "inv_apply", "inv_block", "linear"]

ABI_VERSION = 16
NB = 128
NPAD = 64


class EmcidHipError(RuntimeError):
    pass


def lib_path() -> Path:
    return _LIB_PATH


def load():
    global _lib
    if _lib is not None:
        return _lib
    if not _LIB_PATH.exists():
        raise EmcidHipError(
            f"{_LIB_PATH} is missing: build it with `python -c 'import __graft_entry__ as g; g.build()'` "
            f"or `make -C {_LIB_PATH.parent}`. The MI355X path has no CPU fallback.")
    lib = C.CDLL(str(_LIB_PATH))
    p, i64, i32, f64, f32 = C.c_void_p, C.c_int64, C.c_int, C.c_double, C.c_float
    sig = {
        "emcid_abi_version": (i32, []),
        "emcid_last_error": (C.c_char_p, []),
        "emcid_gram_accumulate_f32": (i32, [p, i64, i64, i64, p, i64, i32, p]),
        "emcid_symmetrize_lower_f32": (i32, [p, i64, i64, p]),
        "emcid_gather_mean_f32": (i32, [p, i64, i64, i64, i64, i64, p, p, i64, p, i64, p]),
        "emcid_edit_workspace_bytes": (i64, [i64, i64, i64]),
        "emcid_edit_layer_f64": (i32, [p, p, p, p, i64, i64, i64, f64, f64, i32, p, p, p, p, p, p, i64, p, p]),
        "emcid_edit_layer_shard_f64": (i32, [p, p, p, p, i64, i64, i64, f64, f64, i32, i64, i64, p, p, p, p, i64, p, p]),
        "emcid_apply_update_f32": (i32, [p, p, p, p, i64, p]),
        "emcid_assemble_spd_f64": (i32, [p, i64, p, i64, i64, i64, f64, f32, p, i64, p]),
        "emcid_cholesky_f64": (i32, [p, p, i64, i64, p, p, p]),
        "emcid_inverse_workspace_doubles": (i64, [i64]),
        "emcid_debug_leaf_stamps": (i32, [p, p, p, p, p, p]),
        "emcid_cov_factor_workspace_bytes": (i64, [i64, i64]),
        "emcid_factor_cov_f64": (i32, [p, i64, i64, f64, f64, p, i64, p, p]),
        "emcid_cov_inverse_f64": (i32, [p, i64, i64, i64, i64, p]),
        "emcid_cov_factor_rescale_f64": (i32, [p, p, i64, i64, i64, f64, i32, p]),
        "emcid_edit_dual_workspace_bytes": (i64, [i64, i64, i64]),
        "emcid_edit_dual_stage1_f64": (i32, [p, p, p, i64, i64, i64, f64, i32, f64, p, i64, i64, i64, i64, i32, p, i64, p]),
        "emcid_edit_dual_pt": (p, [p, i64, i64, i64]),
        "emcid_edit_dual_stage2_f64": (i32, [i64, i64, i64, f64, p, p, p, p, p, p, i64, p, p]),
        "emcid_edit_dual_apply_stage1_f64": (i32, [p, p, p, i64, i64, i64, f64, i32, f64, p, i64, i64, i64, i64, i32, p, i64, p]),
        "emcid_edit_dual_yt": (p, [p, i64, i64, i64]),
        "emcid_edit_dual_apply_stage2_f64": (i32, [i64, i64, i64, p, i64, i64, i32, i32, p, p, p, p, i64, p, p]),
        "emcid_edit_dual_apply_assemble_f64": (i32, [i64, i64, i64, p, i64, p]),
        "emcid_edit_dual_preserve_workspace_bytes": (i64, [i64, i64, i64, i64]),
        "emcid_edit_layer_dual_preserve_f64": (i32, [p, p, p, i64, i64, i64, f64, i32, f64, p, i64, i64, p, i64, p, i64, p, i64, i64,
                                                     p, p, p, p, p, i64, p, p]),
        "emcid_session_retain_workspace_bytes": (i64, [i64, i64, i64]),
        "emcid_session_retain_f64": (i32, [p, i64, i64, f64, f64, p, i64, i64, p, i64, p, i64, p, i64, i64, p, i64, p, p]),
        "emcid_session_step_norms_f64": (i32, [p, i64, i64, i64, i64, i64, i64, p, p, p, p]),
        "emcid_session_release_workspace_bytes": (i64, [i64, i64, i64]),
        "emcid_session_release_f64": (i32, [p, i64, i64, i64, p, i64, p, i64, p, i64, i64, p, i64, p, p]),
        "emcid_cov_factor_fold_workspace_bytes": (i64, [i64, i64]),
        "emcid_cov_factor_fold_f64": (i32, [p, f64, p, i64, i64, i64, p, f64, f64, i32, p, i64, i64, i64, p, p, i64, p, p]),
        "emcid_cholesky_solve_f64": (i32, [p, i64, i64, p, p, p, i64, i64, p]),
        "emcid_edit_dual_cols_stage1_f64": (i32, [p, p, p, i64, i64, i64, f64, i32, f64, p, i64, i64, p, i32, p, i64, p]),
        "emcid_edit_dual_s": (p, [p, i64, i64, i64]),
        "emcid_edit_dual_u": (p, [p, i64, i64, i64]),
        "emcid_edit_dual_cols_stage2_f64": (i32, [i64, i64, i64, p, i64, i64, p, i32, p, i64, p, p]),
        "emcid_apply_update2d_f32": (i32, [p, i64, p, p, p, i64, i64, p]),
        "emcid_edit_lu_workspace_bytes": (i64, [i64, i64, i64]),
        "emcid_edit_layer_lu_f64": (i32, [p, p, p, p, i64, i64, i64, f64, f64, i32, p, p, p, p, p, p, i64, p, p]),
        "emcid_lu_solve_f64": (i32, [p, i64, i64, p, i64, i64, p, p, p]),
        "emcid_delta_w_f64": (i32, [p, i64, p, i64, i64, i64, i64, p, p, i64, p, p, p]),
        "emcid_dgemm_f64": (i32, [i32, i32, i64, i64, i64, f64, p, i64, p, i64, f64, p, i64, p]),
        "emcid_dgemm_ex_f64": (i32, [i32, i32, i64, i64, i64, f64, p, i64, p, i64, f64, p, i64, i32, i32, i32, p]),
        "emcid_dgemm_batched_f64": (i32, [i32, i32, i64, i64, i64, f64, p, i64, i64, p, i64, i64, f64, p, i64, i64, i64, p]),
        "emcid_streamk_workspace_bytes": (i64, [i32]),
        "emcid_debug_streamk_stamps": (i32, [p]),
        "emcid_debug_linear_sp16_stamps": (i32, [p]),
        "emcid_fingerprint_store": (i32, [i64, p, p, p, p, i64, p]),
        "emcid_fingerprint_check": (i32, [p, i64, i64, i64, p, p, p]),
        "emcid_debug_step_stamps": (i32, [p]),
        "emcid_dgemm_streamk_f64": (i32, [i32, i64, i64, i64, f64, p, i64, p, i64, p, i64, i32, i32, f64, p, i64, p]),
        "emcid_axpy_f32": (i32, [p, p, i64, p]),
        "emcid_quick_gelu_f32": (i32, [p, p, i64, p]),
        "emcid_linear_f32": (i32, [p, i64, p, i64, p, p, i64, p, i64, i64, i64, i64, i32, i32, p]),
        "emcid_linear_ws_f32": (i32, [p, i64, p, i64, p, p, i64, p, i64, i64, i64, i64, i32, i32, p, i64, p]),
        "emcid_linear_workspace_bytes": (i64, []),
        "emcid_split_rows_f16": (i32, [p, i64, i64, i64, p, i64, p, p, p]),
        "emcid_gram_sp16_workspace_bytes": (i64, [i64]),
        "emcid_gram_sp16_workspace_bytes_for": (i64, [i64, i64]),
        "emcid_gram_accumulate_sp16_f32": (i32, [p, p, i64, i64, i64, p, i64, p, i64, p]),
        "emcid_add_layernorm_sp16": (i32, [p, i64, p, i64, p, p, C.c_float, i64, i64, p, p, p, i64, p, p, p, p]),
        "emcid_embed_layernorm_sp16": (i32, [p, i64, i64, p, i64, i64, p, p, p, p, C.c_float, i64, i64, p, p, p, i64, p, p]),
        "emcid_tree_attention_sp16_supported": (i32, [i64, i64, i64]),
        "emcid_clip_workspace_bytes": (i64, [i64, i64, i64]),
        "emcid_clip_layer_head_sp16": (i32, [p, i64, i64, i64, i64, f32, p, i64, p, p, i64, p, p, p, p, p, p, p, p, i64, p]),
        "emcid_clip_layer_tail_sp16": (i32, [p, i64, i64, i64, p, p, p, p, p, p, f32, p, p, p]),
        "emcid_clip_layers_sp16": (i32, [p, i64, i64, i64, i64, i64, f32, p, i64, p, p, p, p, p, p, f32, p, i64, p]),
        "emcid_clip_edit_layer_tail_sp16": (i32, [p, i64, i64, i64, p, p, p, p, p, p, i64, i64, p, f64, i32, f64, p, i64, i64, i32,
                                                 p, p, p, p, p, p, p, p, i64, p, p, i64, p, p, p, f32, p, p, p]),
        "emcid_tree_attention_sp16": (i32, [p, i64, p, p, i64, p, i64, p, p, i64, i64, i64, f32, p, i64, p, p]),
        "emcid_linear_sp16_f32": (i32, [p, i64, p, p, i64, p, p, p, i64, p, i64, p, i64, p, i64, i64, i64, i32, i32, p]),
        "emcid_add_layernorm_f32": (i32, [p, i64, p, i64, p, p, C.c_float, i64, i64, p, p, p]),
        "emcid_embed_layernorm_f32": (i32, [p, i64, i64, p, i64, i64, p, p, p, p, C.c_float, i64, i64, p, p, p]),
        "emcid_tree_attention_f32": (i32, [p, i64, p, p, i64, p, i64, p, p, i64, i64, i64, f32, p, i64, p]),
        "emcid_profile_enable": (i32, [C.c_uint]),
        "emcid_profile_collect": (i32, [p, p, i32]),
        "emcid_attention_f32": (i32, [p, p, p, i64, i64, i64, p, i32, i64, i64, i32, f32, i64, i64, i64, i64, p, p]),
    }
    for name, (res, args) in sig.items():
        fn = getattr(lib, name)
        fn.restype, fn.argtypes = res, args
    if lib.emcid_abi_version() != ABI_VERSION:
        raise EmcidHipError(f"ABI mismatch: library {lib.emcid_abi_version()} vs binding {ABI_VERSION}; rebuild csrc/")
    _lib = lib
    return lib


_tls = threading.local()


def _check(rc: int, what: str):
    restore = getattr(_tls, "restore", None)
    if restore:
        torch.cuda.set_device(restore.pop())
    if rc != 0:
        raise EmcidHipError(f"{what} failed (rc={rc}): {load().emcid_last_error().decode()}")


def _ptr(t: Optional[torch.Tensor], dtype=None, what="tensor"):
    if t is None:
        return None
    if not t.is_cuda:
        raise EmcidHipError(f"{what} must live in HBM (got device {t.device}); there is no CPU path")
    if dtype is not None and t.dtype != dtype:
        raise EmcidHipError(f"{what} must be {dtype}, got {t.dtype}")
    return C.c_void_p(t.data_ptr())


def _stream(t: torch.Tensor):
    idx = t.device.index
    cur = torch.cuda.current_device()
    if idx is not None and idx != cur:
        if getattr(_tls, "restore", None) is None:
            _tls.restore = []
        _tls.restore.append(cur)
        torch.cuda.set_device(idx)
    return C.c_void_p(torch.cuda.current_stream(t.device).cuda_stream)



GRAM_SPLIT = os.environ.get("EMCID_GRAM_SPLIT", "1") != "0"
_GRAM_WS = {}


def gram_takes_row_weight(X: torch.Tensor, ksplit: int = 0) -> bool:
    d = X.shape[1]
    return bool(GRAM_SPLIT and ksplit != 1 and X.shape[0] >= 2048 and d % 4 == 0 and d >= 256 and X.stride(0) % 4 == 0
                and X.stride(1) == 1 and X.data_ptr() % 16 == 0 and X.dtype == torch.float32)


def gram_accumulate_(G: torch.Tensor, X: torch.Tensor, ksplit: int = 0, row_weight: Optional[torch.Tensor] = None):
    assert X.dim() == 2 and G.dim() == 2 and G.shape[0] == G.shape[1] == X.shape[1]
    assert X.stride(1) == 1 and G.stride(1) == 1
    if X.shape[0] == 0:
        return G
    d = X.shape[1]
    if row_weight is not None:
        assert row_weight.shape == (X.shape[0],) and row_weight.dtype == torch.float32 and row_weight.is_contiguous()
        if not (gram_takes_row_weight(X, ksplit) and G.dtype == torch.float32):
            X, row_weight = X * row_weight.unsqueeze(1), None
    if GRAM_SPLIT and ksplit != 1 and X.shape[0] >= 2048 and d % 4 == 0 and d >= 256 and X.stride(0) % 4 == 0 \
            and X.data_ptr() % 16 == 0 and X.dtype == torch.float32 and G.dtype == torch.float32:
        key = (X.device.index if X.device.index is not None else torch.cuda.current_device(),
               torch.cuda.current_stream(X.device).cuda_stream, d)
        need = int(load().emcid_gram_sp16_workspace_bytes_for(d, X.shape[0]))
        ws = _GRAM_WS.get(key)
        if ws is None or ws.numel() < need:
            if ws is None and len(_GRAM_WS) >= 8:
                _GRAM_WS.clear()
            ws = _GRAM_WS[key] = torch.empty(need, dtype=torch.uint8, device=X.device)
        _check(load().emcid_gram_accumulate_sp16_f32(_ptr(X, torch.float32, "X"),
                                                     _ptr(row_weight, torch.float32, "row_weight") if row_weight is not None else None,
                                                     X.shape[0], d, X.stride(0),
                                                     _ptr(G, torch.float32, "G"), G.stride(0), C.c_void_p(ws.data_ptr()),
                                                     ws.numel(), _stream(G)), "emcid_gram_accumulate_sp16_f32")
        return G
    _check(load().emcid_gram_accumulate_f32(_ptr(X, torch.float32, "X"), X.shape[0], X.shape[1], X.stride(0),
                                            _ptr(G, torch.float32, "G"), G.stride(0), ksplit, _stream(G)),
           "emcid_gram_accumulate_f32")
    return G


def symmetrize_lower_(G: torch.Tensor):
    _check(load().emcid_symmetrize_lower_f32(_ptr(G, torch.float32, "G"), G.shape[0], G.stride(0), _stream(G)),
           "emcid_symmetrize_lower_f32")
    return G



def gather_mean(act: torch.Tensor, idx: torch.Tensor, seg: torch.Tensor, out: Optional[torch.Tensor] = None):
    assert act.dim() == 3 and act.stride(2) == 1
    B, S, c = act.shape
    N = seg.numel() - 1
    assert idx.numel() == B
    if out is None:
        out = torch.empty(N, c, dtype=torch.float32, device=act.device)
    _check(load().emcid_gather_mean_f32(_ptr(act, torch.float32, "act"), B, S, c, act.stride(0), act.stride(1),
                                        _ptr(idx, torch.int64, "idx"), _ptr(seg, torch.int64, "seg"), N,
                                        _ptr(out, torch.float32, "out"), out.stride(0), _stream(act)),
           "emcid_gather_mean_f32")
    return out



def edit_workspace_bytes(N: int, d: int, h: int) -> int:
    return int(load().emcid_edit_workspace_bytes(N, d, h))


class EditWorkspace:

    def __init__(self, N: int, d: int, h: int, device, lu: bool = False):
        self.key = (N, d, h)
        self.lu = lu
        self.nbytes = int(load().emcid_edit_lu_workspace_bytes(N, d, h)) if lu else edit_workspace_bytes(N, d, h)
        self.buf = torch.zeros(self.nbytes // 8, dtype=torch.float64, device=device)
        self.info = torch.zeros(1, dtype=torch.int32, device=device)


def edit_layer(K, Zc, zs_t, Cov, lam: float, edit_weight: float, layers_left: int, W0=None, W=None,
               want_factors: bool = False, want_dw: bool = True, ws: Optional[EditWorkspace] = None):
    N, d = K.shape
    h = Zc.shape[1]
    assert Cov.shape == (d, d) and zs_t.shape == (N, h) and Zc.shape == (N, h)
    for t, nm in ((K, "K"), (Zc, "Zc"), (zs_t, "zs_t"), (Cov, "C")):
        assert t.is_contiguous(), nm
    if ws is None or ws.key != (N, d, h) or ws.lu:
        ws = EditWorkspace(N, d, h, K.device)
    dev = K.device
    Xt = torch.empty(N, d, dtype=torch.float64, device=dev) if want_factors else None
    Rt = torch.empty(N, h, dtype=torch.float64, device=dev) if want_factors else None
    dW = torch.empty(h, d, dtype=torch.float32, device=dev) if want_dw else None
    if W is not None:
        assert W.is_contiguous() and W.shape == (h, d) and W0 is not None and W0.is_contiguous()
    _check(load().emcid_edit_layer_f64(
        _ptr(K, torch.float32, "K"), _ptr(Zc, torch.float32, "Zc"), _ptr(zs_t, torch.float32, "zs_t"),
        _ptr(Cov, torch.float32, "C"), N, d, h, float(lam), float(edit_weight), int(layers_left),
        _ptr(W0, torch.float32, "W0"), _ptr(W, torch.float32, "W"), _ptr(Xt), _ptr(Rt), _ptr(dW),
        _ptr(ws.buf), ws.nbytes, _ptr(ws.info, torch.int32, "info"), _stream(K)), "emcid_edit_layer_f64")
    return {"Xt": Xt, "Rt": Rt, "dW": dW, "ws": ws}


def edit_layer_lu(K, Zc, zs_t, Cov, lam: float, edit_weight: float, layers_left: int, W0=None, W=None,
                  want_factors: bool = False, want_dw: bool = True, ws: Optional[EditWorkspace] = None):
    N, d = K.shape
    h = Zc.shape[1]
    assert Cov.shape == (d, d) and zs_t.shape == (N, h) and Zc.shape == (N, h)
    for t, nm in ((K, "K"), (Zc, "Zc"), (zs_t, "zs_t"), (Cov, "C")):
        assert t.is_contiguous(), nm
    if ws is None or ws.key != (N, d, h) or not ws.lu:
        ws = EditWorkspace(N, d, h, K.device, lu=True)
    dev = K.device
    adj_k = torch.empty(d, N, dtype=torch.float64, device=dev) if want_factors else None
    Rt = torch.empty(N, h, dtype=torch.float64, device=dev) if want_factors else None
    dW = torch.empty(h, d, dtype=torch.float32, device=dev) if want_dw else None
    if W is not None:
        assert W.is_contiguous() and W.shape == (h, d) and W0 is not None and W0.is_contiguous()
    _check(load().emcid_edit_layer_lu_f64(
        _ptr(K, torch.float32, "K"), _ptr(Zc, torch.float32, "Zc"), _ptr(zs_t, torch.float32, "zs_t"),
        _ptr(Cov, torch.float32, "C"), N, d, h, float(lam), float(edit_weight), int(layers_left),
        _ptr(W0, torch.float32, "W0"), _ptr(W, torch.float32, "W"), _ptr(adj_k), _ptr(Rt), _ptr(dW),
        _ptr(ws.buf), ws.nbytes, _ptr(ws.info, torch.int32, "info"), _stream(K)), "emcid_edit_layer_lu_f64")
    return {"adj_k": adj_k, "Rt": Rt, "dW": dW, "ws": ws}


def lu_solve_(A: torch.Tensor, B: torch.Tensor):
    n = A.shape[0]
    piv = torch.zeros(n, dtype=torch.int32, device=A.device)
    info = torch.zeros(1, dtype=torch.int32, device=A.device)
    _check(load().emcid_lu_solve_f64(_ptr(A, torch.float64, "A"), A.stride(0), n, _ptr(B, torch.float64, "B"), B.stride(0),
                                     B.shape[1], _ptr(piv), _ptr(info), _stream(A)), "emcid_lu_solve_f64")
    return piv, info


def edit_layer_shard(K, Zc, zs_t, Cov, lam: float, edit_weight: float, layers_left: int, rows, want_factors=False,
                     ws: Optional[EditWorkspace] = None):
    N, d = K.shape
    h = Zc.shape[1]
    lo, hi = rows
    assert Cov.shape == (d, d) and zs_t.shape == (N, h) and Zc.shape == (N, h) and 0 <= lo < hi <= N
    for t, nm in ((K, "K"), (Zc, "Zc"), (zs_t, "zs_t"), (Cov, "C")):
        assert t.is_contiguous(), nm
    if ws is None or ws.key != (N, d, h) or ws.lu:
        ws = EditWorkspace(N, d, h, K.device)
    dev = K.device
    U = torch.empty(h, d, dtype=torch.float64, device=dev)
    Xt = torch.empty(hi - lo, d, dtype=torch.float64, device=dev) if want_factors else None
    Rt = torch.empty(hi - lo, h, dtype=torch.float64, device=dev) if want_factors else None
    _check(load().emcid_edit_layer_shard_f64(
        _ptr(K, torch.float32, "K"), _ptr(Zc, torch.float32, "Zc"), _ptr(zs_t, torch.float32, "zs_t"),
        _ptr(Cov, torch.float32, "C"), N, d, h, float(lam), float(edit_weight), int(layers_left), lo, hi,
        _ptr(U), _ptr(Xt), _ptr(Rt), _ptr(ws.buf), ws.nbytes, _ptr(ws.info, torch.int32, "info"), _stream(K)),
        "emcid_edit_layer_shard_f64")
    return {"U": U, "Xt": Xt, "Rt": Rt, "ws": ws}
# ... 493 lines not shown
        C.c_void_p(base), rows, h, d, heads, float(scale), _ptr(anc, torch.int32, "anc"), anc.stride(0),
        _ptr(depth, torch.int32, "depth"), _ptr(rows_sel, torch.int32, "rows") if rows_sel is not None else None, n,
        _ptr(hs, torch.float32, "hs"), _ptr(x.planes), _ptr(x.inv_scale), _ptr(mid), _ptr(f_planes), _ptr(f_scale), _ptr(f_f32),
        C.c_void_p(ws.data_ptr()), ws.numel(), _stream(hs)), "emcid_clip_layer_head_sp16")
    return mid, SplitRows(f_planes, f_scale[1], f_f32)


def clip_layer_tail(layer_array, index: int, h: int, d: int, f: "SplitRows", mid: torch.Tensor,
                    next_ln: Optional[torch.nn.LayerNorm]):
    dev = mid.device
    n = mid.shape[0]
    hs = torch.empty(n, h, dtype=torch.float32, device=dev)
    x = None
    if next_ln is not None:
        x = SplitRows(torch.empty(n, h, dtype=torch.int32, device=dev), torch.empty(n, dtype=torch.float32, device=dev))
    if LINEAR_FLOPS["count"]:
        LINEAR_FLOPS["flops"] += 2.0 * n * h * d
        LINEAR_FLOPS["launches"] += 1
    base = C.addressof(layer_array) + index * C.sizeof(ClipLayerSp16)
    _check(load().emcid_clip_layer_tail_sp16(
        C.c_void_p(base), n, h, d, _ptr(f.planes), _ptr(f.inv_scale), _ptr(mid, torch.float32, "mid"), _ptr(hs),
        _ptr(next_ln.weight, torch.float32, "gamma") if next_ln is not None else None,
        _ptr(next_ln.bias, torch.float32, "beta") if next_ln is not None else None,
        float(next_ln.eps) if next_ln is not None else 0.0, _ptr(x.planes) if x is not None else None,
        _ptr(x.inv_scale) if x is not None else None, _stream(mid)), "emcid_clip_layer_tail_sp16")
    return hs, x


def clip_edit_layer_tail(layer_array, index: int, h: int, d: int, f: "SplitRows", mid: torch.Tensor, lookup: torch.Tensor,
                         seg: torch.Tensor, zs_t: torch.Tensor, factors: "CovFactors", layer_index: int, edit_weight: float,
                         layers_left: int, W0: torch.Tensor, W: torch.Tensor, ws: "DualWorkspace", lam: Optional[float],
                         next_ln: Optional[torch.nn.LayerNorm], last: bool, want_dw: bool = True, zc_split: bool = True):
    dev = mid.device
    n = f.f32.shape[0]
    N = seg.numel() - 1
    K = torch.empty(N, d, dtype=torch.float32, device=dev)
    Zc = torch.empty(N, h, dtype=torch.float32, device=dev)
    dW = torch.empty(h, d, dtype=torch.float32, device=dev) if want_dw else None
    kp = torch.empty(N, d, dtype=torch.int32, device=dev) if zc_split else None
    ks = torch.empty(N, dtype=torch.float32, device=dev) if zc_split else None
    hs = x = None
    if not last:
        hs = torch.empty(n, h, dtype=torch.float32, device=dev)
        if next_ln is not None:
            x = SplitRows(torch.empty(n, h, dtype=torch.int32, device=dev), torch.empty(n, dtype=torch.float32, device=dev))
    lws = _linear_workspace(dev) if (d >= 2048 and -(-N // 128) * -(-h // 128) <= 128
                                     and not torch.cuda.is_current_stream_capturing()) else None
    if LINEAR_FLOPS["count"]:
        LINEAR_FLOPS["flops"] += 2.0 * N * h * d + (0.0 if last else 2.0 * n * h * d)
        LINEAR_FLOPS["launches"] += 1 if last else 2
    base = C.addressof(layer_array) + index * C.sizeof(ClipLayerSp16)
    use_inverse = layer_index in factors.have_inverse
    _check(load().emcid_clip_edit_layer_tail_sp16(
        C.c_void_p(base), n, h, d, _ptr(f.f32, torch.float32, "fc2 input"), _ptr(f.planes), _ptr(f.inv_scale),
        _ptr(mid, torch.float32, "mid"), _ptr(lookup, torch.int64, "lookup"), _ptr(seg, torch.int64, "seg"), lookup.numel(), N,
        _ptr(zs_t, torch.float32, "zs_t"), float(edit_weight), int(layers_left), factors.lam_ratio(lam), _ptr(factors.buf),
        factors.n_layers, int(layer_index), int(bool(use_inverse)), _ptr(W0, torch.float32, "W0"), _ptr(W, torch.float32, "W"),
        _ptr(dW), _ptr(K), _ptr(Zc), _ptr(kp), _ptr(ks), _ptr(ws.buf), ws.nbytes, _ptr(ws.info, torch.int32),
        C.c_void_p(lws.data_ptr()) if lws is not None else None, lws.numel() if lws is not None else 0, _ptr(hs),
        _ptr(next_ln.weight, torch.float32, "gamma") if (next_ln is not None and not last) else None,
        _ptr(next_ln.bias, torch.float32, "beta") if (next_ln is not None and not last) else None,
        float(next_ln.eps) if (next_ln is not None and not last) else 0.0, _ptr(x.planes) if x is not None else None,
        _ptr(x.inv_scale) if x is not None else None, _stream(mid)), "emcid_clip_edit_layer_tail_sp16")
    return {"K": K, "Zc": Zc, "dW": dW, "hs": hs, "x": x}



class CovFactors:

    def __init__(self, n_layers: int, d: int, device):
        self.n_layers, self.d = n_layers, d
        self.nbytes = int(load().emcid_cov_factor_workspace_bytes(n_layers, d))
        self.buf = torch.zeros(self.nbytes // 8, dtype=torch.float64, device=device)
        self.info = torch.zeros(1, dtype=torch.int32, device=device)
        self.dp = (d + NB - 1) // NB * NB
        self._inv = ((self.dp + 511) // 512) * (512 * 512 + 256 * 256)
        self.have_inverse = set()
        self.ready = None
        self.cached = False
        self.lam = None
        self.edit_weight = None

    def lam_ratio(self, lam: Optional[float]) -> float:
        if lam is None or self.lam is None or float(lam) == self.lam:
            return 1.0
        if not (lam > 0.0 and self.lam > 0.0):
            raise EmcidHipError(f"mom2_update_weight must be positive for the Cholesky path (got {lam})")
        return float(lam) / float(self.lam)

    def L(self, layer: int) -> torch.Tensor:
        o = (self.n_layers + layer) * self.dp * self.dp
        return self.buf[o:o + self.dp * self.dp].view(self.dp, self.dp)

    def X(self, layer: int) -> torch.Tensor:
        o = self.n_layers * (2 * self.dp * self.dp + self._inv) + layer * self.dp * self.dp
        return self.buf[o:o + self.dp * self.dp].view(self.dp, self.dp)


def cov_inverse(factors: "CovFactors", first: int = 0, count: Optional[int] = None):
    count = factors.n_layers - first if count is None else count
    _check(load().emcid_cov_inverse_f64(_ptr(factors.buf), factors.n_layers, factors.d, int(first), int(count),
                                        _stream(factors.buf)), "emcid_cov_inverse_f64")
    factors.have_inverse.update(range(first, first + count))


def factor_cov(covs, lam: float, edit_weight: float, factors: Optional[CovFactors] = None, inverse: bool = True) -> CovFactors:
    d = covs[0].shape[0]
    for c in covs:
        assert c.shape == (d, d) and c.is_contiguous()
    if factors is None or factors.n_layers != len(covs) or factors.d != d:
        factors = CovFactors(len(covs), d, covs[0].device)
    arr = (C.c_void_p * len(covs))(*[_ptr(c, torch.float32, "C").value for c in covs])
    _check(load().emcid_factor_cov_f64(arr, len(covs), d, float(lam), float(edit_weight), _ptr(factors.buf), factors.nbytes,
                                       _ptr(factors.info, torch.int32), _stream(covs[0])), "emcid_factor_cov_f64")
    factors.have_inverse = set()
    factors.lam, factors.edit_weight = float(lam), float(edit_weight)
    if inverse:
        cov_inverse(factors)
    return factors


def cov_factor_rescale(src: CovFactors, a: float, dst: Optional[CovFactors] = None, lam: Optional[float] = None,
                       edit_weight: Optional[float] = None) -> CovFactors:
    if not (a > 0.0 and a < 1e300):
        raise EmcidHipError(f"the scale of a factored workspace must be positive and finite (got {a})")
    with_inverse = len(src.have_inverse) == src.n_layers
    if dst is None or dst.n_layers != src.n_layers or dst.d != src.d or dst.buf.device != src.buf.device:
        dst = CovFactors(src.n_layers, src.d, src.buf.device)
    if dst is not src:
        dst.info.zero_()
    _check(load().emcid_cov_factor_rescale_f64(_ptr(src.buf), _ptr(dst.buf), dst.nbytes, src.n_layers, src.d, float(a),
                                               int(with_inverse), _stream(src.buf)), "emcid_cov_factor_rescale_f64")
    dst.have_inverse = set(range(src.n_layers)) if with_inverse else set()
    dst.lam = float(lam) if lam is not None else (src.lam * float(a) if src.lam is not None else None)
    dst.edit_weight = float(edit_weight) if edit_weight is not None else src.edit_weight
    return dst


class DualWorkspace:
    def __init__(self, N: int, d: int, h: int, device):
        self.key = (N, d, h)
        self.nbytes = int(load().emcid_edit_dual_workspace_bytes(N, d, h))
        self.buf = torch.zeros(self.nbytes // 8, dtype=torch.float64, device=device)
        self.info = torch.zeros(1, dtype=torch.int32, device=device)
        self.Np, self.dp = (N + NB - 1) // NB * NB, (d + NB - 1) // NB * NB
        pt = load().emcid_edit_dual_pt(_ptr(self.buf), N, d, h)
        off = (pt - self.buf.data_ptr()) // 8
        self.Pt = self.buf[off:off + self.Np * self.dp].view(self.Np, self.dp)
        hp = h + (h % 2)
        off = (load().emcid_edit_dual_s(_ptr(self.buf), N, d, h) - self.buf.data_ptr()) // 8
        self.S = self.buf[off:off + self.Np * self.Np].view(self.Np, self.Np)
        off = (load().emcid_edit_dual_u(_ptr(self.buf), N, d, h) - self.buf.data_ptr()) // 8
        self.U = self.buf[off:off + hp * self.dp].view(hp, self.dp)[:h]


def edit_layer_dual(K, Zc, zs_t, factors: CovFactors, layer_index: int, edit_weight: float, layers_left: int,
                    W0=None, W=None, want_factors: bool = False, want_dw: bool = True, ws: Optional[DualWorkspace] = None,
                    rows=None, gather_pt=None, use_inverse: Optional[bool] = None, lam: Optional[float] = None):
    if use_inverse is None:
        use_inverse = layer_index in factors.have_inverse
    N, d = K.shape
    h = Zc.shape[1]
    for t, nm in ((K, "K"), (Zc, "Zc"), (zs_t, "zs_t")):
        assert t.is_contiguous(), nm
    assert zs_t.shape == (N, h) and factors.d == d
    if ws is None or ws.key != (N, d, h):
        ws = DualWorkspace(N, d, h, K.device)
    lo, hi = rows if rows is not None else (0, N)
    lib = load()
    _check(lib.emcid_edit_dual_stage1_f64(
        _ptr(K, torch.float32, "K"), _ptr(Zc, torch.float32, "Zc"), _ptr(zs_t, torch.float32, "zs_t"), N, d, h,
        float(edit_weight), int(layers_left), factors.lam_ratio(lam), _ptr(factors.buf), factors.n_layers, int(layer_index), lo, hi,
        int(bool(use_inverse)), _ptr(ws.buf), ws.nbytes, _stream(K)), "emcid_edit_dual_stage1_f64")
    if gather_pt is not None:
        ws.Pt[:N].copy_(gather_pt(ws.Pt[lo:hi]))
    dev = K.device
    adj_k = torch.empty(d, N, dtype=torch.float64, device=dev) if want_factors else None
    Rt = torch.empty(N, h, dtype=torch.float64, device=dev) if want_factors else None
    dW = torch.empty(h, d, dtype=torch.float32, device=dev) if want_dw else None
    if W is not None:
        assert W.is_contiguous() and W.shape == (h, d) and W0 is not None and W0.is_contiguous()
    _check(lib.emcid_edit_dual_stage2_f64(N, d, h, factors.lam_ratio(lam), _ptr(W0, torch.float32, "W0"), _ptr(W, torch.float32, "W"), _ptr(adj_k),
                                          _ptr(Rt), _ptr(dW), _ptr(ws.buf), ws.nbytes, _ptr(ws.info, torch.int32),
                                          _stream(K)), "emcid_edit_dual_stage2_f64")
    return {"adj_k": adj_k, "Rt": Rt, "dW": dW, "ws": ws}


def column_tiles(rank: int, world: int, n_tiles: int):
    load_ = [0] * world
    owner = {}
    for t in range(n_tiles - 1, -1, -1):
        r = min(range(world), key=lambda i: (load_[i], i))
        owner[t] = r
        load_[r] += t + 1
    return [t for t in range(n_tiles) if owner[t] == rank]


class _HipColsBackend:

    def __init__(self, K, Zc, zs_t, factors, layer_index, edit_weight, layers_left, ws, lam=None):
        self.a = (K, Zc, zs_t, factors, layer_index, edit_weight, layers_left, ws)
        self.lam_ratio = factors.lam_ratio(lam)

    def stage1(self, tiles):
        K, Zc, zs_t, factors, layer_index, edit_weight, layers_left, ws = self.a
        N, d = K.shape
        arr = (C.c_int * len(tiles))(*tiles)
        _check(load().emcid_edit_dual_cols_stage1_f64(
            _ptr(K, torch.float32, "K"), _ptr(Zc, torch.float32, "Zc"), _ptr(zs_t, torch.float32, "zs_t"), N, d, Zc.shape[1],
            float(edit_weight), int(layers_left), self.lam_ratio, _ptr(factors.buf), factors.n_layers, int(layer_index), arr,
            len(tiles), _ptr(ws.buf), ws.nbytes, _stream(K)), "emcid_edit_dual_cols_stage1_f64")
        return ws.S

    def stage2(self, tiles):
        K, Zc, zs_t, factors, layer_index, edit_weight, layers_left, ws = self.a
        N, d = K.shape
        arr = (C.c_int * len(tiles))(*tiles)
        _check(load().emcid_edit_dual_cols_stage2_f64(N, d, Zc.shape[1], _ptr(factors.buf), factors.n_layers, int(layer_index), arr,
                                                      len(tiles), _ptr(ws.buf), ws.nbytes, _ptr(ws.info, torch.int32), _stream(K)),
               "emcid_edit_dual_cols_stage2_f64")
        return ws.U

    def apply(self, U, W0, W, want_dw):
        K, Zc = self.a[0], self.a[1]
        h, d = Zc.shape[1], K.shape[1]
        dW = torch.empty(h, d, dtype=torch.float32, device=K.device) if want_dw else None
        _check(load().emcid_apply_update2d_f32(_ptr(U), U.stride(0), _ptr(W0, torch.float32, "W0"), _ptr(W, torch.float32, "W"),
                                               _ptr(dW), h, d, _stream(K)), "emcid_apply_update2d_f32")
        return dW


def edit_layer_dual_cols(K, Zc, zs_t, factors, layer_index: int, edit_weight: float, layers_left: int, W0, W,
                         tiles, all_reduce, want_dw: bool = True, ws: Optional["DualWorkspace"] = None, backend=None,
                         lam: Optional[float] = None):
    N, d = K.shape
    h = Zc.shape[1]
    tiles = sorted(int(t) for t in tiles)
    if not tiles:
        raise EmcidHipError("a rank without a column tile: world size exceeds d / 128")
    if backend is None:
        for t, nm in ((K, "K"), (Zc, "Zc"), (zs_t, "zs_t"), (W, "W"), (W0, "W0")):
            assert t.is_contiguous(), nm
        assert zs_t.shape == (N, h) and factors.d == d and W.shape == (h, d)
        if layer_index not in factors.have_inverse:
            raise EmcidHipError("edit_layer_dual_cols needs the explicit inverse factor of the layer (cov_inverse)")
        if ws is None or ws.key != (N, d, h):
            ws = DualWorkspace(N, d, h, K.device)
        backend = _HipColsBackend(K, Zc, zs_t, factors, layer_index, edit_weight, layers_left, ws, lam)
    S = backend.stage1(tiles)
    all_reduce(S)
    U = backend.stage2(tiles)
    all_reduce(U)
    dW = backend.apply(U, W0, W, want_dw)
    return {"dW": dW, "ws": ws}


def edit_layer_dual_apply(K, Zc, zs_t, factors: CovFactors, layer_index: int, edit_weight: float, layers_left: int,
                          W0, W, want_dw: bool = True, ws: Optional[DualWorkspace] = None,
                          use_inverse: Optional[bool] = None, on_factor_start=None, lam: Optional[float] = None):
    if use_inverse is None:
        use_inverse = layer_index in factors.have_inverse
    N, d = K.shape
    h = Zc.shape[1]
    for t, nm in ((K, "K"), (Zc, "Zc"), (zs_t, "zs_t"), (W, "W"), (W0, "W0")):
        assert t.is_contiguous(), nm
    assert zs_t.shape == (N, h) and factors.d == d and W.shape == (h, d)
    if ws is None or ws.key != (N, d, h):
        ws = DualWorkspace(N, d, h, K.device)
    lib = load()
    _check(lib.emcid_edit_dual_apply_stage1_f64(
        _ptr(K, torch.float32, "K"), _ptr(Zc, torch.float32, "Zc"), _ptr(zs_t, torch.float32, "zs_t"), N, d, h,
        float(edit_weight), int(layers_left), factors.lam_ratio(lam), _ptr(factors.buf), factors.n_layers, int(layer_index), 0, N,
        int(bool(use_inverse)), _ptr(ws.buf), ws.nbytes, _stream(K)), "emcid_edit_dual_apply_stage1_f64")
    dW = torch.empty(h, d, dtype=torch.float32, device=K.device) if want_dw else None
    if on_factor_start is not None:
        _check(lib.emcid_edit_dual_apply_assemble_f64(N, d, h, _ptr(ws.buf), ws.nbytes, _stream(K)),
               "emcid_edit_dual_apply_assemble_f64")
        on_factor_start()
    _check(lib.emcid_edit_dual_apply_stage2_f64(N, d, h, _ptr(factors.buf), factors.n_layers, int(layer_index),
                                                int(bool(use_inverse)), int(on_factor_start is not None),
                                                _ptr(W0, torch.float32, "W0"), _ptr(W, torch.float32, "W"), _ptr(dW),
                                                _ptr(ws.buf), ws.nbytes, _ptr(ws.info, torch.int32), _stream(K)),
           "emcid_edit_dual_apply_stage2_f64")
    return {"dW": dW, "ws": ws}


class PreservedKeys:

    def __init__(self, n_layers: int, d: int, capacity: int, device):
        if capacity < 1:
            raise EmcidHipError(f"the capacity of a preserved key set must be positive (got {capacity})")
        self.n_layers, self.d, self.capacity, self.M = int(n_layers), int(d), int(capacity), 0
        self.dp = (d + NB - 1) // NB * NB
        self.ldl = self.capacity + (self.capacity % 2)
        tiles = (self.capacity + NB - 1) // NB
        self.Yp = [torch.zeros(self.capacity, self.dp, dtype=torch.float64, device=device) for _ in range(n_layers)]
        self.Lp = [torch.zeros(self.capacity, self.ldl, dtype=torch.float64, device=device) for _ in range(n_layers)]
        self.tile_inv = [torch.zeros(tiles, NB, NB, dtype=torch.float64, device=device) for _ in range(n_layers)]
        self.row_scale = torch.ones(self.capacity, dtype=torch.float64)

    def commit(self, N: int, scale: float = 1.0):
        assert self.M + N <= self.capacity
        self.row_scale[self.M:self.M + int(N)] = float(scale)
        self.M += int(N)

    def release_commit(self, keep):
        keep = check_keep(keep, self.M)[0]
        self.row_scale[:len(keep)] = self.row_scale[torch.as_tensor(keep, dtype=torch.long)]
        self.M = len(keep)

    def reset(self):
        self.M = 0

    def check_layer(self, layer_index: int):
        if not 0 <= layer_index < self.n_layers:
            raise EmcidHipError(f"layer index {layer_index} outside the session state's {self.n_layers} layers")

    def layer_args(self, layer_index: int):
        self.check_layer(layer_index)
        Yp, Lp, Ti = self.Yp[layer_index], self.Lp[layer_index], self.tile_inv[layer_index]
        for t, nm in ((Yp, "Yp"), (Lp, "Lp"), (Ti, "tile_inv")):
            assert t.stride(-1) == 1 and (t.dim() < 3 or t.is_contiguous()), nm
        return (_ptr(Yp, torch.float64, "Yp"), Yp.stride(0), _ptr(Lp, torch.float64, "Lp"), Lp.stride(0),
                _ptr(Ti, torch.float64, "tile_inv"), self.capacity, self.M)

    @property
    def nbytes(self) -> int:
        return sum(t.numel() * 8 for ts in (self.Yp, self.Lp, self.tile_inv) for t in ts)


class _SessionWorkspace:

    def __init__(self, what: str, size_fn, dims: dict, device):
        self.key = tuple(dims.values())
        self.nbytes = int(size_fn(*self.key))
        if self.nbytes <= 0:
            raise EmcidHipError(f"no {what} workspace for " + ", ".join(f"{k}={v}" for k, v in dims.items()))
        self.buf = torch.zeros(self.nbytes // 8, dtype=torch.float64, device=device)
        self.info = torch.zeros(1, dtype=torch.int32, device=device)


class PreserveWorkspace(_SessionWorkspace):

    def __init__(self, N: int, d: int, h: int, capacity: int, device):
        super().__init__("preserve", load().emcid_edit_dual_preserve_workspace_bytes, dict(N=N, d=d, h=h, capacity=capacity), device)


class RetainWorkspace(_SessionWorkspace):

    def __init__(self, N: int, d: int, capacity: int, device):
        super().__init__("retain", load().emcid_session_retain_workspace_bytes, dict(N=N, d=d, capacity=capacity), device)


class ReleaseWorkspace(_SessionWorkspace):

    def __init__(self, n_rebuilt: int, d: int, capacity: int, device):
        super().__init__("release", load().emcid_session_release_workspace_bytes, dict(n_rebuilt=n_rebuilt, d=d, capacity=capacity),
                         device)


def edit_layer_dual_preserve(K, Zc, zs_t, factors: CovFactors, layer_index: int, edit_weight: float, layers_left: int,
                             W0, W, state: PreservedKeys, want_dw: bool = True, want_u: bool = False,
                             ws: Optional[PreserveWorkspace] = None, lam: Optional[float] = None):
    N, d = K.shape
    h = Zc.shape[1]
    for t, nm in ((K, "K"), (Zc, "Zc"), (zs_t, "zs_t")) + (((W, "W"), (W0, "W0")) if W is not None else ()):
        assert t.is_contiguous(), nm
    assert zs_t.shape == (N, h) and factors.d == d == state.d and (W is None or W.shape == (h, d))
    state.check_layer(layer_index)
    if layer_index not in factors.have_inverse:
        raise EmcidHipError("edit_layer_dual_preserve needs the explicit inverse factor of the layer (cov_inverse)")
    if state.M + N > state.capacity:
        raise EmcidHipError(f"{state.M} preserved + {N} new rows exceed the state's capacity {state.capacity}")
    if ws is None or ws.key != (N, d, h, state.capacity):
        ws = PreserveWorkspace(N, d, h, state.capacity, K.device)
    dW = torch.empty(h, d, dtype=torch.float32, device=K.device) if want_dw else None
    U = torch.empty(h, d, dtype=torch.float64, device=K.device) if want_u else None
    _check(load().emcid_edit_layer_dual_preserve_f64(
        _ptr(K, torch.float32, "K"), _ptr(Zc, torch.float32, "Zc"), _ptr(zs_t, torch.float32, "zs_t"), N, d, h,
        float(edit_weight), int(layers_left), factors.lam_ratio(lam), _ptr(factors.buf), factors.n_layers, int(layer_index),
        *state.layer_args(layer_index), _ptr(W0, torch.float32, "W0"), _ptr(W, torch.float32, "W"), _ptr(dW), _ptr(U),
        _ptr(ws.buf), ws.nbytes, _ptr(ws.info, torch.int32), _stream(K)), "emcid_edit_layer_dual_preserve_f64")
    return {"dW": dW, "U": U, "ws": ws}


def row_scale_of(edit_weight: float, factors: CovFactors, lam: Optional[float] = None, weight: float = 1.0) -> float:
    return math.sqrt(float(weight) * float(edit_weight) / 0.5) / math.sqrt(factors.lam_ratio(lam))


def session_retain(K, factors: CovFactors, layer_index: int, row_scale: float, state: PreservedKeys,
                   ws: Optional[RetainWorkspace] = None, lam: Optional[float] = None):
    N, d = K.shape
    assert K.is_contiguous(), "K"
    assert factors.d == d == state.d
    state.check_layer(layer_index)
    if layer_index not in factors.have_inverse:
        raise EmcidHipError("session_retain needs the explicit inverse factor of the layer (cov_inverse)")
    if state.M + N > state.capacity:
        raise EmcidHipError(f"{state.M} preserved + {N} retained rows exceed the state's capacity {state.capacity}")
    row_scale = float(row_scale)
    if not (row_scale > 0.0 and row_scale < float("inf")):
        raise EmcidHipError(f"row_scale must be positive and finite (got {row_scale})")
    if ws is None or ws.key != (N, d, state.capacity):
        ws = RetainWorkspace(N, d, state.capacity, K.device)
    _check(load().emcid_session_retain_f64(
        _ptr(K, torch.float32, "K"), N, d, row_scale, factors.lam_ratio(lam), _ptr(factors.buf), factors.n_layers, int(layer_index),
        *state.layer_args(layer_index), _ptr(ws.buf), ws.nbytes, _ptr(ws.info, torch.int32), _stream(K)), "emcid_session_retain_f64")
    return {"ws": ws}


def check_keep(keep, M: int):
    keep = [int(i) for i in keep]
    if any(i < 0 or i >= M for i in keep) or any(b <= a for a, b in zip(keep, keep[1:])):
        raise EmcidHipError(f"keep must be strictly ascending row indices inside [0, {M})")
    first = next((j for j, i in enumerate(keep) if i != j), len(keep))
    return keep, first


def session_release(state: PreservedKeys, layer_index: int, keep, first: Optional[int] = None, ws: Optional[ReleaseWorkspace] = None):
    state.check_layer(layer_index)
    Yp = state.Yp[layer_index]
    if isinstance(keep, torch.Tensor) and keep.is_cuda:
        if first is None:
            raise EmcidHipError("session_release: a device tensor of kept rows needs `first`")
        keep_dev, n_keep, first = keep, int(keep.numel()), int(first)
        if keep_dev.dtype != torch.int32 or not keep_dev.is_contiguous() or keep_dev.device != Yp.device:
            raise EmcidHipError(f"session_release: keep must be a contiguous int32 tensor on {Yp.device}")
    else:
        rows, f = check_keep(keep.tolist() if isinstance(keep, torch.Tensor) else keep, state.M)
        if first is not None and int(first) != f:
            raise EmcidHipError(f"session_release: first = {first}, but the smallest released row of keep is {f}")
        keep_dev, n_keep, first = None, len(rows), f
    if not 0 <= first <= n_keep <= state.M:
        raise EmcidHipError(f"session_release: first = {first}, {n_keep} kept rows, {state.M} committed")
    if n_keep == state.M or first == n_keep:
        return {"ws": None, "launched": False, "first": first}
# ... 63 lines not shown
```

### include/emcid_hip.h

```cpp
#ifndef EMCID_HIP_H
#define EMCID_HIP_H

#include <stdint.h>

#ifdef __cplusplus
extern "C" {
#endif

#define EMCID_OK 0
#define EMCID_ERR_BAD_ARG (-1)
#define EMCID_ERR_HIP (-2)
#define EMCID_ERR_WORKSPACE (-3)

#define EMCID_ABI_VERSION 16

int emcid_abi_version(void);
const char* emcid_last_error(void);

#define EMCID_PROF_CLASSES 16
int emcid_profile_enable(unsigned class_mask);
int emcid_profile_collect(double* ms_per_class_host, int64_t* launches_per_class_host, int n_classes);

int emcid_gram_accumulate_f32(const float* X, int64_t t, int64_t d, int64_t ldx,
                              float* G, int64_t ldg, int ksplit, void* stream);
int emcid_symmetrize_lower_f32(float* G, int64_t d, int64_t ldg, void* stream);

int emcid_gather_mean_f32(const float* act, int64_t B, int64_t S, int64_t c, int64_t ldb, int64_t lds_,
                          const int64_t* idx, const int64_t* seg, int64_t N,
                          float* out, int64_t ldo, void* stream);

int emcid_attention_f32(const float* q, const float* k, const float* v, int64_t sb, int64_t sh, int64_t ss,
                        const void* mask, int mask_kind, int64_t mb, int64_t mi, int causal, float scale,
                        int64_t B, int64_t H, int64_t S, int64_t D, float* out, void* stream);

int emcid_tree_attention_f32(const float* q, int64_t ldq, const float* k, const float* v, int64_t ld, const int* anc, int64_t anc_ld,
                             const int* depth, const int* rows, int64_t n_rows, int64_t H, int64_t D, float scale,
                             float* out, int64_t ldo, void* stream);

int emcid_quick_gelu_f32(const float* x, float* y, int64_t n, void* stream);

int emcid_linear_f32(const float* X, int64_t ldx, const float* W, int64_t ldw, const float* bias, const float* residual,
                     int64_t ldr, float* Y, int64_t ldy, int64_t M, int64_t N, int64_t K, int act, int cfg, void* stream);

int64_t emcid_linear_workspace_bytes(void);
int emcid_linear_ws_f32(const float* X, int64_t ldx, const float* W, int64_t ldw, const float* bias, const float* residual,
                        int64_t ldr, float* Y, int64_t ldy, int64_t M, int64_t N, int64_t K, int act, int cfg, void* workspace,
                        int64_t workspace_bytes, void* stream);

int emcid_split_rows_f16(const float* X, int64_t ldx, int64_t rows, int64_t K, void* planes, int64_t ldp, float* inv_scale,
                         float* max_row_norm, void* stream);

int emcid_linear_sp16_f32(const void* Xp, int64_t ldx, const float* x_inv_scale, const void* Wp, int64_t ldw,
                          const float* w_inv_scale, const float* bias, const float* residual, int64_t ldr, float* Y, int64_t ldy,
                          void* Yp, int64_t ldp, const float* y_scale, int64_t M, int64_t N, int64_t K, int act, int cfg,
                          void* stream);

int emcid_debug_linear_sp16_stamps(long long* stamps_dev);
int64_t emcid_gram_sp16_workspace_bytes(int64_t d);
int64_t emcid_gram_sp16_workspace_bytes_for(int64_t d, int64_t t);
int emcid_gram_accumulate_sp16_f32(const float* X, const float* row_weight, int64_t t, int64_t d, int64_t ldx, float* G, int64_t ldg,
                                   void* workspace, int64_t workspace_bytes, void* stream);

int emcid_add_layernorm_sp16(const float* a, int64_t lda, const float* b, int64_t ldb, const float* gamma, const float* beta,
                             float eps, int64_t rows, int64_t cols, float* y, float* z, void* planes, int64_t ldp,
                             float* inv_scale, const float* bound, float* out_scale, void* stream);
int emcid_embed_layernorm_sp16(const float* tok, int64_t ld_tok, int64_t n_tok, const float* pos, int64_t ld_pos, int64_t n_pos,
                               const int64_t* token, const int* position, const float* gamma, const float* beta, float eps,
                               int64_t rows, int64_t cols, float* y, float* z, void* planes, int64_t ldp, float* inv_scale,
                               void* stream);
int emcid_tree_attention_sp16_supported(int64_t anc_ld, int64_t H, int64_t D);
int emcid_tree_attention_sp16(const float* q, int64_t ldq, const float* k, const float* v, int64_t ld, const int* anc,
                              int64_t anc_ld, const int* depth, const int* rows, int64_t n_rows, int64_t H, int64_t D, float scale,
                              void* planes, int64_t ldp, float* inv_scale, void* stream);

int emcid_fingerprint_store(int64_t n, const void* const* data, const int64_t* bytes, const int64_t* slots, void* table,
                            int64_t table_slots, void* stream);
int emcid_fingerprint_check(const void* table, int64_t table_slots, int64_t first_slot, int64_t n_slots, const uint64_t* skip_mask,
                            int* flag, void* stream);

typedef struct emcid_clip_layer_sp16 {
    const float* ln1_gamma; const float* ln1_beta;
    const float* ln2_gamma; const float* ln2_beta;
    const void* qkv_planes; const float* qkv_inv_scale; const float* qkv_bias;
    const void* out_planes; const float* out_inv_scale; const float* out_bias;
    const void* fc1_planes; const float* fc1_inv_scale; const float* fc1_bias; const float* fc1_bound;
    const void* fc2_planes; const float* fc2_inv_scale; const float* fc2_bias;
    float ln1_eps, ln2_eps;
    int32_t act, reserved;
} emcid_clip_layer_sp16;

int64_t emcid_clip_workspace_bytes(int64_t rows, int64_t h, int64_t d);

int emcid_clip_layer_head_sp16(const emcid_clip_layer_sp16* L, int64_t rows, int64_t h, int64_t d, int64_t heads, float attn_scale,
                               const int* anc, int64_t anc_ld, const int* depth, const int* rows_sel, int64_t n_sel,
                               const float* hs, const void* x_planes, const float* x_inv_scale, float* mid, void* f_planes,
                               float* f_scale, float* f_f32, void* workspace, int64_t workspace_bytes, void* stream);

int emcid_clip_layer_tail_sp16(const emcid_clip_layer_sp16* L, int64_t n, int64_t h, int64_t d, const void* f_planes,
                               const float* f_inv_scale, const float* mid, float* hs_out, const float* next_ln_gamma,
                               const float* next_ln_beta, float next_ln_eps, void* x_planes, float* x_inv_scale, void* stream);

int emcid_clip_edit_layer_tail_sp16(const emcid_clip_layer_sp16* L, int64_t n_rows, int64_t h, int64_t d, const float* f_f32,
                                    const void* f_planes, const float* f_inv_scale, const float* mid, const int64_t* lookup,
                                    const int64_t* seg, int64_t B, int64_t N, const float* zs_t, double edit_weight,
                                    int layers_left, double lam_ratio, const void* cov_factor_ws, int64_t n_layers,
                                    int64_t layer_index, int use_inverse, const float* W0, float* W, float* dW, float* K_out,
                                    float* Zc_out, void* k_planes, float* k_inv_scale, void* dual_ws, int64_t dual_ws_bytes,
                                    int* info_dev, void* linear_ws, int64_t linear_ws_bytes, float* hs_out,
                                    const float* next_ln_gamma, const float* next_ln_beta, float next_ln_eps, void* x_planes,
                                    float* x_inv_scale, void* stream);

int emcid_clip_layers_sp16(const emcid_clip_layer_sp16* layers, int64_t n_layers, int64_t rows, int64_t h, int64_t d, int64_t heads,
                           float attn_scale, const int* anc, int64_t anc_ld, const int* depth, float* hs, void* x_planes,
                           float* x_inv_scale, const float* next_ln_gamma, const float* next_ln_beta, float next_ln_eps,
                           void* workspace, int64_t workspace_bytes, void* stream);

int emcid_add_layernorm_f32(const float* a, int64_t lda, const float* b, int64_t ldb, const float* gamma, const float* beta,
                            float eps, int64_t rows, int64_t cols, float* y, float* z, void* stream);

int emcid_embed_layernorm_f32(const float* tok, int64_t ld_tok, int64_t n_tok, const float* pos, int64_t ld_pos, int64_t n_pos,
                              const int64_t* token, const int* position, const float* gamma, const float* beta, float eps,
                              int64_t rows, int64_t cols, float* y, float* z, void* stream);

int64_t emcid_edit_workspace_bytes(int64_t N, int64_t d, int64_t h);

int emcid_edit_layer_f64(const float* K, const float* Zc, const float* zs_t, const float* C,
                         int64_t N, int64_t d, int64_t h,
                         double lam, double edit_weight, int layers_left,
                         const float* W0, float* W,
                         double* Xt_out, double* Rt_out, float* dW_out,
                         void* workspace, int64_t workspace_bytes, int* info_dev, void* stream);
int emcid_cov_inverse_f64(void* cov_factor_ws, int64_t n_layers, int64_t d, int64_t first_layer, int64_t count, void* stream);

int emcid_edit_layer_shard_f64(const float* K, const float* Zc, const float* zs_t, const float* C,
                               int64_t N, int64_t d, int64_t h, double lam, double edit_weight, int layers_left,
                               int64_t n_lo, int64_t n_hi, double* U_partial, double* Xt_out, double* Rt_out,
                               void* workspace, int64_t workspace_bytes, int* info_dev, void* stream);
int emcid_apply_update_f32(const double* U, const float* W0, float* W, float* dW, int64_t n, void* stream);

int64_t emcid_cov_factor_workspace_bytes(int64_t n_layers, int64_t d);
int emcid_factor_cov_f64(const float* const* C_host_list, int64_t n_layers, int64_t d, double lam, double edit_weight,
                         void* workspace, int64_t workspace_bytes, int* info_dev, void* stream);
int emcid_cov_factor_rescale_f64(const void* src_ws, void* dst_ws, int64_t workspace_bytes, int64_t n_layers, int64_t d, double a,
                                 int with_inverse, void* stream);
int64_t emcid_edit_dual_workspace_bytes(int64_t N, int64_t d, int64_t h);
int emcid_edit_dual_stage1_f64(const float* K, const float* Zc, const float* zs_t, int64_t N, int64_t d, int64_t h,
                               double edit_weight, int layers_left, double lam_ratio, const void* cov_factor_ws, int64_t n_layers,
                               int64_t layer_index, int64_t n_lo, int64_t n_hi, int use_inverse, void* workspace,
                               int64_t workspace_bytes, void* stream);
double* emcid_edit_dual_pt(void* workspace, int64_t N, int64_t d, int64_t h);
int emcid_edit_dual_stage2_f64(int64_t N, int64_t d, int64_t h, double lam_ratio, const float* W0, float* W, double* adjk_out, double* Rt_out,
                               float* dW_out, void* workspace, int64_t workspace_bytes, int* info_dev, void* stream);

int emcid_edit_dual_apply_stage1_f64(const float* K, const float* Zc, const float* zs_t, int64_t N, int64_t d, int64_t h,
                                     double edit_weight, int layers_left, double lam_ratio, const void* cov_factor_ws, int64_t n_layers,
                                     int64_t layer_index, int64_t n_lo, int64_t n_hi, int use_inverse, void* workspace,
                                     int64_t workspace_bytes, void* stream);
double* emcid_edit_dual_yt(void* workspace, int64_t N, int64_t d, int64_t h);
int emcid_edit_dual_apply_stage2_f64(int64_t N, int64_t d, int64_t h, const void* cov_factor_ws, int64_t n_layers,
                                     int64_t layer_index, int use_inverse, int assembled, const float* W0, float* W,
                                     float* dW_out, void* workspace, int64_t workspace_bytes, int* info_dev, void* stream);
int emcid_edit_dual_apply_assemble_f64(int64_t N, int64_t d, int64_t h, void* workspace, int64_t workspace_bytes, void* stream);

int64_t emcid_edit_dual_preserve_workspace_bytes(int64_t N, int64_t d, int64_t h, int64_t capacity);
int emcid_edit_layer_dual_preserve_f64(const float* K, const float* Zc, const float* zs_t, int64_t N, int64_t d, int64_t h,
                                       double edit_weight, int layers_left, double lam_ratio, const void* cov_factor_ws,
                                       int64_t n_layers, int64_t layer_index, double* Yp, int64_t ldy, double* Lp, int64_t ldl,
                                       double* tile_inv, int64_t capacity, int64_t M, const float* W0, float* W, float* dW_out,
                                       double* U_out, void* workspace, int64_t workspace_bytes, int* info_dev, void* stream);

int64_t emcid_session_retain_workspace_bytes(int64_t N, int64_t d, int64_t capacity);
int emcid_session_retain_f64(const float* K, int64_t N, int64_t d, double row_scale, double lam_ratio, const void* cov_factor_ws,
                             int64_t n_layers, int64_t layer_index, double* Yp, int64_t ldy, double* Lp, int64_t ldl,
                             double* tile_inv, int64_t capacity, int64_t M, void* workspace, int64_t workspace_bytes, int* info_dev,
                             void* stream);

int64_t emcid_session_release_workspace_bytes(int64_t n_rebuilt, int64_t d, int64_t capacity);
int emcid_session_release_f64(const int32_t* keep_dev, int64_t n_keep, int64_t first, int64_t d, double* Yp, int64_t ldy, double* Lp,
                              int64_t ldl, double* tile_inv, int64_t capacity, int64_t M, void* workspace, int64_t workspace_bytes,
                              int* info_dev, void* stream);

int emcid_session_step_norms_f64(const void* workspace, int64_t workspace_bytes, int64_t N, int64_t d, int64_t h, int64_t capacity,
                                 int64_t M, double* drift_out, double* left_out, double* resid_out, void* stream);

int64_t emcid_cov_factor_fold_workspace_bytes(int64_t M, int64_t d);
int emcid_cov_factor_fold_f64(const void* src_ws, double lam_ratio, const double* Yp, int64_t ldy, int64_t M, int64_t capacity,
                              const float* C, double lam, double edit_weight, int fill_base, void* dst_ws, int64_t n_layers,
                              int64_t d, int64_t layer_index, double* base, void* workspace, int64_t workspace_bytes,
                              int* info_dev, void* stream);

int64_t emcid_edit_lu_workspace_bytes(int64_t N, int64_t d, int64_t h);
int emcid_edit_layer_lu_f64(const float* K, const float* Zc, const float* zs_t, const float* C,
                            int64_t N, int64_t d, int64_t h, double lam, double edit_weight, int layers_left,
                            const float* W0, float* W, double* adjk_out, double* Rt_out, float* dW_out,
                            void* workspace, int64_t workspace_bytes, int* info_dev, void* stream);
int emcid_lu_solve_f64(double* A, int64_t lda, int64_t n, double* B, int64_t ldb, int64_t nrhs, int* piv_dev,
                       int* info_dev, void* stream);

int emcid_edit_dual_cols_stage1_f64(const float* K, const float* Zc, const float* zs_t, int64_t N, int64_t d, int64_t h,
                                    double edit_weight, int layers_left, double lam_ratio, const void* cov_factor_ws, int64_t n_layers,
                                    int64_t layer_index, const int* tiles_host, int n_tiles, void* workspace,
                                    int64_t workspace_bytes, void* stream);
double* emcid_edit_dual_s(void* workspace, int64_t N, int64_t d, int64_t h);
double* emcid_edit_dual_u(void* workspace, int64_t N, int64_t d, int64_t h);
int emcid_edit_dual_cols_stage2_f64(int64_t N, int64_t d, int64_t h, const void* cov_factor_ws, int64_t n_layers,
                                    int64_t layer_index, const int* tiles_host, int n_tiles, void* workspace,
                                    int64_t workspace_bytes, int* info_dev, void* stream);
int emcid_apply_update2d_f32(const double* U, int64_t ldu, const float* W0, float* W, float* dW, int64_t h, int64_t d,
                             void* stream);


int emcid_assemble_spd_f64(const float* C, int64_t ldc, const double* Kt64, int64_t Np, int64_t d, int64_t ldk,
                           double lam, float cw, double* A, int64_t lda, void* stream);
int64_t emcid_inverse_workspace_doubles(int64_t dp);
int emcid_debug_leaf_stamps(const double* A, double* L, double* inv, int* info_dev, long long* stamps_dev, void* stream);
int emcid_cholesky_f64(double* A, double* L, int64_t dp, int64_t lda, double* invdiag, int* info_dev, void* stream);
int emcid_cholesky_solve_f64(const double* L, int64_t dp, int64_t lda, const double* invdiag,
                             double* Bt, double* Yt, int64_t Np, int64_t ldb, void* stream);
int emcid_delta_w_f64(const double* Rt, int64_t ldr, const double* Xt, int64_t ldx, int64_t Np, int64_t h, int64_t d,
                      const float* W0, float* W, int64_t ldw, float* dW, double* U, void* stream);

int emcid_dgemm_f64(int ta, int tb, int64_t M, int64_t N, int64_t K, double alpha,
                    const double* A, int64_t lda, const double* B, int64_t ldb,
                    double beta, double* C, int64_t ldc, void* stream);
int emcid_dgemm_ex_f64(int ta, int tb, int64_t M, int64_t N, int64_t K, double alpha,
                       const double* A, int64_t lda, const double* B, int64_t ldb,
                       double beta, double* C, int64_t ldc, int flags, int cfg, int ksplit, void* stream);

int64_t emcid_streamk_workspace_bytes(int wgs);
int emcid_dgemm_streamk_f64(int tb, int64_t M, int64_t N, int64_t K, double alpha, const double* A, int64_t lda,
                            const double* B, int64_t ldb, double* C, int64_t ldc, int flags, int wgs, double diag_add,
                            void* workspace, int64_t workspace_bytes, void* stream);

int emcid_debug_streamk_stamps(long long* stamps_dev);
int emcid_debug_step_stamps(long long* stamps_dev);

int emcid_dgemm_batched_f64(int ta, int tb, int64_t M, int64_t N, int64_t K, double alpha,
                            const double* A, int64_t lda, int64_t sA, const double* B, int64_t ldb, int64_t sB,
                            double beta, double* C, int64_t ldc, int64_t sC, int64_t batch, void* stream);

int emcid_axpy_f32(float* W, const float* dW, int64_t n, void* stream);

#ifdef __cplusplus
}
#endif
#endif
```

Measured before the change: 111,800.

## Fuse key gather-mean, fp16 split and f64 scaling; write residual pre-transposed

Adds an edit_keys kernel that computes the per-concept mean key, writes the fp32 key, the scaled f64 Kt block and the fp16 split planes in a single pass, replacing separate gather-mean, split and prep kernels. Also adds a prep_rt kernel that writes the residual directly in transposed form, so the Schur RHS solve skips its transpose. This cuts several launches and intermediate round trips through memory on the edit path, at the cost of more code paths and a d<=8192 limit behind an env flag.

Result: no change. 111,500, median of 3 (-0.3%).

```diff
diff --git a/emcid_amd/csrc/clip_layers.hip b/emcid_amd/csrc/clip_layers.hip
--- a/emcid_amd/csrc/clip_layers.hip
+++ b/emcid_amd/csrc/clip_layers.hip
@@ -213,6 +213,16 @@
     return EMCID_OK;
 }
 
+static int edit_layer_forward_tail(const emcid_clip_layer_sp16* L, int64_t n_rows, int64_t h, int64_t d, const void* f_planes,
+                                   const float* f_inv_scale, const float* mid, const float* W, float* hs_out,
+                                   const float* next_ln_gamma, const float* next_ln_beta, float next_ln_eps, void* x_planes,
+                                   float* x_inv_scale, void* stream) {
+    if (hs_out == nullptr) return EMCID_OK;
+    EMCID_TRY(emcid_split_rows_f16(W, d, h, d, const_cast<void*>(L->fc2_planes), d, const_cast<float*>(L->fc2_inv_scale), nullptr, stream));
+    return emcid_clip_layer_tail_sp16(L, n_rows, h, d, f_planes, f_inv_scale, mid, hs_out, next_ln_gamma, next_ln_beta, next_ln_eps,
+                                      x_planes, x_inv_scale, stream);
+}
+
 int emcid_clip_edit_layer_tail_sp16(const emcid_clip_layer_sp16* L, int64_t n_rows, int64_t h, int64_t d, const float* f_f32,
                                     const void* f_planes, const float* f_inv_scale, const float* mid, const int64_t* lookup,
                                     const int64_t* seg, int64_t B, int64_t N, const float* zs_t, double edit_weight,
@@ -224,8 +234,21 @@
                                     float* x_inv_scale, void* stream) {
     EMCID_CHECK_ARG(L && n_rows > 0 && h % 32 == 0 && d % 32 == 0 && f_f32 && lookup && seg && B > 0 && N > 0 && zs_t);
     EMCID_CHECK_ARG(cov_factor_ws && W0 && W && K_out && Zc_out && dual_ws && info_dev && (hs_out == nullptr || (f_planes && f_inv_scale && mid)));
+    EMCID_CHECK_ARG((k_planes == nullptr) == (k_inv_scale == nullptr));
+    static const int fused_keys = env_flag("EMCID_FUSED_KEYS", 1);
+    if (fused_keys && k_planes != nullptr && d <= 8192) {
+        EMCID_TRY(emcid_edit_keys_f64(f_f32, n_rows, lookup, seg, B, N, d, h, edit_weight, lam_ratio, K_out, k_planes, k_inv_scale,
+                                      dual_ws, dual_ws_bytes, stream));
+        EMCID_TRY(emcid_linear_sp16_f32(k_planes, d, k_inv_scale, L->fc2_planes, d, L->fc2_inv_scale, L->fc2_bias, nullptr, 0, Zc_out, h,
+                                        nullptr, 0, nullptr, N, h, d, 0, -1, stream));
+        EMCID_TRY(emcid_edit_dual_apply_stage1_rt_f64(nullptr, Zc_out, zs_t, N, d, h, edit_weight, layers_left, lam_ratio, cov_factor_ws,
+                                                      n_layers, layer_index, 0, N, use_inverse, dual_ws, dual_ws_bytes, stream));
+        EMCID_TRY(emcid_edit_dual_apply_stage2_rt_f64(N, d, h, cov_factor_ws, n_layers, layer_index, use_inverse, 0, W0, W, dW, dual_ws,
+                                                      dual_ws_bytes, info_dev, stream));
+        return edit_layer_forward_tail(L, n_rows, h, d, f_planes, f_inv_scale, mid, W, hs_out, next_ln_gamma, next_ln_beta, next_ln_eps,
+                                       x_planes, x_inv_scale, stream);
+    }
     EMCID_TRY(emcid_gather_mean_f32(f_f32, B, n_rows, d, 0, d, lookup, seg, N, K_out, d, stream));
-    EMCID_CHECK_ARG((k_planes == nullptr) == (k_inv_scale == nullptr));
     if (k_planes != nullptr) {
         EMCID_TRY(emcid_split_rows_f16(K_out, d, N, d, k_planes, d, k_inv_scale, nullptr, stream));
         EMCID_TRY(emcid_linear_sp16_f32(k_planes, d, k_inv_scale, L->fc2_planes, d, L->fc2_inv_scale, L->fc2_bias, nullptr, 0, Zc_out, h,
@@ -237,13 +260,8 @@
                                                n_layers, layer_index, 0, N, use_inverse, dual_ws, dual_ws_bytes, stream));
     EMCID_TRY(emcid_edit_dual_apply_stage2_f64(N, d, h, cov_factor_ws, n_layers, layer_index, use_inverse, 0, W0, W, dW, dual_ws,
                                                dual_ws_bytes, info_dev, stream));
-    if (hs_out != nullptr) {
-        EMCID_TRY(emcid_split_rows_f16(W, d, h, d, const_cast<void*>(L->fc2_planes), d, const_cast<float*>(L->fc2_inv_scale), nullptr,
-                                       stream));
-        EMCID_TRY(emcid_clip_layer_tail_sp16(L, n_rows, h, d, f_planes, f_inv_scale, mid, hs_out, next_ln_gamma, next_ln_beta,
-                                             next_ln_eps, x_planes, x_inv_scale, stream));
-    }
-    return EMCID_OK;
+    return edit_layer_forward_tail(L, n_rows, h, d, f_planes, f_inv_scale, mid, W, hs_out, next_ln_gamma, next_ln_beta, next_ln_eps,
+                                   x_planes, x_inv_scale, stream);
 }
 
 int emcid_clip_layers_sp16(const emcid_clip_layer_sp16* layers, int64_t n_layers, int64_t rows, int64_t h, int64_t d, int64_t heads,
diff --git a/emcid_amd/csrc/edit_solve.hip b/emcid_amd/csrc/edit_solve.hip
--- a/emcid_amd/csrc/edit_solve.hip
+++ b/emcid_amd/csrc/edit_solve.hip
@@ -1,4 +1,5 @@
 #include "spd_solve.h"
+#include "sp16.h"
 
 namespace emcid {
 
@@ -99,6 +100,101 @@
     __syncthreads();
     for (int r = ty; r < 32; r += 8)
         if (bx + r < cols && by + tx < rows) dst[(int64_t)(bx + r) * ldd + by + tx] = tile[tx][r];
+}
+
+template <int G>
+__global__ __launch_bounds__(256) void edit_keys_kernel(const float* __restrict__ act, int64_t S, const int64_t* __restrict__ idx,
+                                                         const int64_t* __restrict__ seg, int N, int d, int dp, double s, double g,
+                                                         float* __restrict__ K_out, uint32_t* __restrict__ P,
+                                                         float* __restrict__ inv_scale, double* __restrict__ Kt64) {
+    typedef double v2d __attribute__((ext_vector_type(2)));
+    const int n = blockIdx.x, tid = threadIdx.x;
+    double* kt = Kt64 + (int64_t)n * dp;
+    if (n >= N) {
+        for (int j = 2 * tid; j < dp; j += 512) *reinterpret_cast<v2d*>(kt + j) = (v2d){0.0, 0.0};
+        return;
+    }
+    const int ng = d / 8;
+    const int64_t p0 = seg[n], p1 = seg[n + 1];
+    sp_v4f a[G], b[G];
+#pragma unroll
+    for (int u = 0; u < G; ++u) a[u] = b[u] = (sp_v4f){0.f, 0.f, 0.f, 0.f};
+    for (int64_t p = p0; p < p1; ++p) {
+        int64_t r = idx[p];
+        r = r < 0 ? 0 : (r >= S ? S - 1 : r);
+        const float* x = act + r * d;
+#pragma unroll
+        for (int u = 0; u < G; ++u) {
+            const int gi = tid + 256 * u;
+            if (gi < ng) {
+                a[u] += *reinterpret_cast<const sp_v4f*>(x + 8 * gi);
+                b[u] += *reinterpret_cast<const sp_v4f*>(x + 8 * gi + 4);
+            }
+        }
+    }
+    const float cnt = (float)(p1 - p0);
+    float amax = 0.f;
+#pragma unroll
+    for (int u = 0; u < G; ++u) {
+        const int gi = tid + 256 * u;
+        if (gi < ng) {
+#pragma unroll
+            for (int e = 0; e < 4; ++e) {
+                a[u][e] = (p1 > p0) ? a[u][e] / cnt : 0.f;
+                b[u][e] = (p1 > p0) ? b[u][e] / cnt : 0.f;
+                amax = fmaxf(amax, fmaxf(fabsf(a[u][e]), fabsf(b[u][e])));
+            }
+            float* ko = K_out + (int64_t)n * d + 8 * gi;
+            *reinterpret_cast<sp_v4f*>(ko) = a[u];
+            *reinterpret_cast<sp_v4f*>(ko + 4) = b[u];
+#pragma unroll
+            for (int e = 0; e < 4; e += 2) {
+                *reinterpret_cast<v2d*>(kt + 8 * gi + e) = (v2d){(double)a[u][e] * s * g, (double)a[u][e + 1] * s * g};
+                *reinterpret_cast<v2d*>(kt + 8 * gi + 4 + e) = (v2d){(double)b[u][e] * s * g, (double)b[u][e + 1] * s * g};
+            }
+        }
+    }
+    for (int j = d + 2 * tid; j < dp; j += 512) *reinterpret_cast<v2d*>(kt + j) = (v2d){0.0, 0.0};
+    __shared__ float red[4];
+#pragma unroll
+    for (int o = 32; o > 0; o >>= 1) amax = fmaxf(amax, __shfl_xor(amax, o, 64));
+    if ((tid & 63) == 0) red[tid >> 6] = amax;
+    __syncthreads();
+    amax = fmaxf(fmaxf(red[0], red[1]), fmaxf(red[2], red[3]));
+    float sc, inv;
+    sp_scale_of(amax, sc, inv);
+    if (tid == 0) inv_scale[n] = inv;
+    uint32_t* pr = P + (int64_t)n * d;
+#pragma unroll
+    for (int u = 0; u < G; ++u) {
+        const int gi = tid + 256 * u;
+        if (gi < ng) {
+            sp_v4u hi, lo;
+            sp_split8(a[u], b[u], sc, hi, lo);
+            *reinterpret_cast<sp_v4u*>(pr + 8 * gi) = hi;
+            *reinterpret_cast<sp_v4u*>(pr + 8 * gi + 4) = lo;
+        }
+    }
+}
+
+__global__ __launch_bounds__(256) void prep_rt_kernel(const float* __restrict__ Zc, const float* __restrict__ zs_t, int N, int h,
+                                                       double s, double layers_left, double g, double* __restrict__ RT, int Np,
+                                                       int hp) {
+    __shared__ double tile[32][33];
+    const int bx = blockIdx.x * 32, by = blockIdx.y * 32;
+    const int tx = threadIdx.x & 31, ty = threadIdx.x >> 5;
+    for (int r = ty; r < 32; r += 8) {
+        const int n = by + r, i = bx + tx;
+        double v = 0.0;
+        if (n < N && i < h) {
+            const float src = zs_t[(int64_t)n * h + i] - Zc[(int64_t)n * h + i];
+            v = ((double)src * s) / layers_left * g;
+        }
+        tile[r][tx] = v;
+    }
+    __syncthreads();
+    for (int r = ty; r < 32; r += 8)
+        if (bx + r < hp && by + tx < Np) RT[(int64_t)(bx + r) * Np + by + tx] = tile[tx][r];
 }
 
 struct EditWorkspace {
@@ -120,9 +216,10 @@
 };
 
 int solve_schur_rhs(const double* R, int64_t hp, int64_t h, int64_t Np, const double* LS, const double* invS, const double* XT,
-                    double* full_inv, double* RT, double* Y2, hipStream_t st) {
-    hipLaunchKernelGGL(transpose_f64_kernel, dim3((unsigned)((hp + 31) / 32), (unsigned)(Np / 32)), dim3(256), 0, st, R, hp, RT, Np,
-                       (int)Np, (int)hp);
+                    double* full_inv, double* RT, double* Y2, hipStream_t st, bool rt_filled) {
+    if (!rt_filled)
+        hipLaunchKernelGGL(transpose_f64_kernel, dim3((unsigned)((hp + 31) / 32), (unsigned)(Np / 32)), dim3(256), 0, st, R, hp, RT,
+                           Np, (int)Np, (int)hp);
     if (XT) {
         ScopedProf sp(KC_TRSM_DIAG, st);
         GemmShape f{RT, Np, XT, Np, (int)h, (int)Np, (int)Np, 0};
@@ -429,20 +526,25 @@
     return EMCID_OK;
 }
 
-int emcid_edit_dual_apply_stage1_f64(const float* K, const float* Zc, const float* zs_t, int64_t N, int64_t d, int64_t h,
-                                     double edit_weight, int layers_left, double lam_ratio, const void* cov_factor_ws, int64_t n_layers,
-                                     int64_t layer_index, int64_t n_lo, int64_t n_hi, int use_inverse, void* workspace,
-                                     int64_t workspace_bytes, void* stream) {
-    EMCID_CHECK_DUAL_STAGE1_ARGS();
+static int dual_apply_stage1_launch(const float* K, const float* Zc, const float* zs_t, int64_t N, int64_t d, int64_t h,
+                                    double edit_weight, int layers_left, double lam_ratio, const void* cov_factor_ws, int64_t n_layers,
+                                    int64_t layer_index, int64_t n_lo, int64_t n_hi, int use_inverse, void* workspace, bool rt_form,
+                                    hipStream_t st) {
     DualWorkspace ws(N, d, h);
-    EMCID_CHECK_WORKSPACE(workspace_bytes, ws.total * (int64_t)sizeof(double), "");
-    hipStream_t st = (hipStream_t)stream;
     double* base = (double*)workspace;
     double *Kt = base + ws.off_K, *Bs = base + ws.off_P, *Yt = base + ws.off_Y, *R = base + ws.off_R;
     const int64_t dp = ws.dp;
     const CovFactorLayout cov(n_layers, d);
     const double *Lb = cov.L(cov_factor_ws, layer_index), *Ib = cov.I(cov_factor_ws, layer_index);
-    launch_prep_kr(K, Zc, zs_t, N, d, h, edit_weight, layers_left, 1.0 / sqrt(lam_ratio), Kt, ws.Np, dp, R, ws.hp, st);
+    const double gain = 1.0 / sqrt(lam_ratio);
+    if (!rt_form) {
+        launch_prep_kr(K, Zc, zs_t, N, d, h, edit_weight, layers_left, gain, Kt, ws.Np, dp, R, ws.hp, st);
+    } else {
+        if (K != nullptr) launch_prep_kr(K, nullptr, nullptr, N, d, h, edit_weight, layers_left, gain, Kt, ws.Np, dp, nullptr, ws.hp, st);
+        ScopedProf sp(KC_PREP, st);
+        hipLaunchKernelGGL(prep_rt_kernel, dim3((unsigned)((ws.hp + 31) / 32), (unsigned)(ws.Np / 32)), dim3(256), 0, st, Zc, zs_t,
+                           (int)N, (int)h, sqrt(edit_weight / 0.5), (double)layers_left, gain, base + ws.off_PT, (int)ws.Np, (int)ws.hp);
+    }
     const int64_t rows = n_hi - n_lo;
     if (use_inverse) {
         const int64_t gemm_rows = (n_lo == 0 && n_hi == N) ? ws.Np : rows;
@@ -462,6 +564,50 @@
     });
 }
 
+int emcid_edit_dual_apply_stage1_f64(const float* K, const float* Zc, const float* zs_t, int64_t N, int64_t d, int64_t h,
+                                     double edit_weight, int layers_left, double lam_ratio, const void* cov_factor_ws, int64_t n_layers,
+                                     int64_t layer_index, int64_t n_lo, int64_t n_hi, int use_inverse, void* workspace,
+                                     int64_t workspace_bytes, void* stream) {
+    EMCID_CHECK_DUAL_STAGE1_ARGS();
+    EMCID_CHECK_WORKSPACE(workspace_bytes, DualWorkspace(N, d, h).total * (int64_t)sizeof(double), "");
+    return dual_apply_stage1_launch(K, Zc, zs_t, N, d, h, edit_weight, layers_left, lam_ratio, cov_factor_ws, n_layers, layer_index,
+                                    n_lo, n_hi, use_inverse, workspace, false, (hipStream_t)stream);
+}
+
+int emcid_edit_keys_f64(const float* act, int64_t n_rows, const int64_t* lookup, const int64_t* seg, int64_t B, int64_t N, int64_t d,
+                        int64_t h, double edit_weight, double lam_ratio, float* K_out, void* k_planes, float* k_inv_scale,
+                        void* workspace, int64_t workspace_bytes, void* stream) {
+    EMCID_CHECK_ARG(act && lookup && seg && K_out && k_planes && k_inv_scale && workspace && n_rows > 0 && B > 0 && N > 0 && h > 0);
+    EMCID_CHECK_ARG(d > 0 && d % 8 == 0 && d <= 8192 && N < (1 << 24) && lam_ratio > 0.0 && lam_ratio < 1e300);
+    EMCID_CHECK_ARG(aligned16(act) && aligned16(K_out) && aligned16(k_planes) && aligned16(workspace));
+    DualWorkspace ws(N, d, h);
+    EMCID_CHECK_WORKSPACE(workspace_bytes, ws.total * (int64_t)sizeof(double), "");
+    hipStream_t st = (hipStream_t)stream;
+    const double s = sqrt(edit_weight / 0.5), g = 1.0 / sqrt(lam_ratio);
+    ScopedProf sp(KC_GATHER, st);
+#define EMCID_EDIT_KEYS(G_)                                                                                                        \
+    hipLaunchKernelGGL(edit_keys_kernel<G_>, dim3((unsigned)ws.Np), dim3(256), 0, st, act, n_rows, lookup, seg, (int)N, (int)d,    \
+                       (int)ws.dp, s, g, K_out, (uint32_t*)k_planes, k_inv_scale, (double*)workspace + ws.off_K)
+    if (d <= 2048) EMCID_EDIT_KEYS(1);
+    else if (d <= 4096) EMCID_EDIT_KEYS(2);
+    else EMCID_EDIT_KEYS(4);
+#undef EMCID_EDIT_KEYS
+    EMCID_CHECK_LAUNCH();
+    return EMCID_OK;
+}
+
+int emcid_edit_dual_apply_stage1_rt_f64(const float* K, const float* Zc, const float* zs_t, int64_t N, int64_t d, int64_t h,
+                                        double edit_weight, int layers_left, double lam_ratio, const void* cov_factor_ws,
+                                        int64_t n_layers, int64_t layer_index, int64_t n_lo, int64_t n_hi, int use_inverse,
+                                        void* workspace, int64_t workspace_bytes, void* stream) {
+    EMCID_CHECK_ARG(Zc && zs_t && N > 0 && d > 0 && h > 0 && layers_left > 0 && cov_factor_ws && workspace);
+    EMCID_CHECK_ARG(0 <= layer_index && layer_index < n_layers && 0 <= n_lo && n_lo < n_hi && n_hi <= N);
+    EMCID_CHECK_ARG(lam_ratio > 0.0 && lam_ratio < 1e300);
+    EMCID_CHECK_WORKSPACE(workspace_bytes, DualWorkspace(N, d, h).total * (int64_t)sizeof(double), "");
+    return dual_apply_stage1_launch(K, Zc, zs_t, N, d, h, edit_weight, layers_left, lam_ratio, cov_factor_ws, n_layers, layer_index,
+                                    n_lo, n_hi, use_inverse, workspace, true, (hipStream_t)stream);
+}
+
 double* emcid_edit_dual_yt(void* workspace, int64_t N, int64_t d, int64_t h) { return dual_block(workspace, N, d, h, &DualWorkspace::off_Y); }
 
 int emcid_edit_dual_apply_assemble_f64(int64_t N, int64_t d, int64_t h, void* workspace, int64_t workspace_bytes, void* stream) {
@@ -477,14 +623,15 @@
     return EMCID_OK;
 }
 
-int emcid_edit_dual_apply_stage2_f64(int64_t N, int64_t d, int64_t h, const void* cov_factor_ws, int64_t n_layers,
-                                     int64_t layer_index, int use_inverse, int assembled, const float* W0, float* W,
-                                     float* dW_out, void* workspace, int64_t workspace_bytes, int* info_dev, void* stream) {
-    EMCID_CHECK_ARG(N > 0 && d > 0 && h > 0 && workspace && info_dev && cov_factor_ws && ((W == nullptr) || (W0 != nullptr)));
-    EMCID_CHECK_ARG(0 <= layer_index && layer_index < n_layers && (W || dW_out));
+#define EMCID_CHECK_APPLY_STAGE2_ARGS()                                                                                              \
+    EMCID_CHECK_ARG(N > 0 && d > 0 && h > 0 && workspace && info_dev && cov_factor_ws && ((W == nullptr) || (W0 != nullptr)));       \
+    EMCID_CHECK_ARG(0 <= layer_index && layer_index < n_layers && (W || dW_out));                                                    \
+    EMCID_CHECK_WORKSPACE(workspace_bytes, DualWorkspace(N, d, h).total * (int64_t)sizeof(double), "")
+
+static int dual_apply_stage2_launch(int64_t N, int64_t d, int64_t h, const void* cov_factor_ws, int64_t n_layers, int64_t layer_index,
+                                    int use_inverse, int assembled, const float* W0, float* W, float* dW_out, void* workspace,
+                                    int* info_dev, bool rt_filled, hipStream_t st) {
     DualWorkspace ws(N, d, h);
-    EMCID_CHECK_WORKSPACE(workspace_bytes, ws.total * (int64_t)sizeof(double), "");
-    hipStream_t st = (hipStream_t)stream;
     double* base = (double*)workspace;
     double *Yt = base + ws.off_Y, *R = base + ws.off_R, *S = base + ws.off_S, *LS = base + ws.off_LS, *invS = base + ws.off_invS;
     double *RT = base + ws.off_PT, *Y2 = base + ws.off_Y2, *V = base + ws.off_V, *U = base + ws.off_U;
@@ -506,7 +653,8 @@
     double *XT = base + ws.off_XT, *TT = base + ws.off_TT;
     EMCID_TRY(with_graph(make_key(GRAPH_APPLY_STAGE2, {Yt, R, S, LS, RT, V, U, info_dev},
                                   {dp, Np, N, hp, (int64_t)(uintptr_t)Lb,
-                                   use_inverse + 2 * (assembled != 0) + 4 * (int)shadow + 8 * h + ((int64_t)p_first << 31) + ((int64_t)xrow << 30) + (d << 32)}),
+                                   use_inverse + 2 * (assembled != 0) + 4 * (int)shadow + 8 * h + ((int64_t)p_first << 31) + ((int64_t)xrow << 30) +
+                                       ((int64_t)rt_filled << 29) + (d << 32)}),
                          st,
                          [&](hipStream_t q) {
         if (!assembled) {
@@ -517,7 +665,7 @@
         job.wgs = (int)((Np + SH_BM - 1) / SH_BM) * (int)(((dp + SH_BN - 1) / SH_BN + 1) / 2);
         const XrowJob xj{XT, Np, TT};
         EMCID_TRY(cholesky_impl(S, LS, Np, Np, invS, info_dev, q, shadow ? &job : nullptr, xrow ? &xj : nullptr));
-        EMCID_TRY(solve_schur_rhs(R, hp, h, Np, LS, invS, xrow ? XT : nullptr, S, RT, Y2, q));
+        EMCID_TRY(solve_schur_rhs(R, hp, h, Np, LS, invS, xrow ? XT : nullptr, S, RT, Y2, q, rt_filled));
         if (!shadow && !p_first) {
             ScopedProf sp(KC_DELTA_W, q);
             GemmShape g{RT, Np, Yt, dp, (int)h, (int)dp, (int)Np, 0};
@@ -539,6 +687,28 @@
     EMCID_CHECK_LAUNCH();
     return EMCID_OK;
 }
+
+int emcid_edit_dual_apply_stage2_f64(int64_t N, int64_t d, int64_t h, const void* cov_factor_ws, int64_t n_layers,
+                                     int64_t layer_index, int use_inverse, int assembled, const float* W0, float* W,
+                                     float* dW_out, void* workspace, int64_t workspace_bytes, int* info_dev, void* stream) {
+    EMCID_CHECK_APPLY_STAGE2_ARGS();
+    return dual_apply_stage2_launch(N, d, h, cov_factor_ws, n_layers, layer_index, use_inverse, assembled, W0, W, dW_out, workspace,
+                                    info_dev, false, (hipStream_t)stream);
+}
+
+int emcid_edit_dual_apply_stage2_rt_f64(int64_t N, int64_t d, int64_t h, const void* cov_factor_ws, int64_t n_layers,
+                                        int64_t layer_index, int use_inverse, int assembled, const float* W0, float* W,
+                                        float* dW_out, void* workspace, int64_t workspace_bytes, int* info_dev, void* stream) {
+    EMCID_CHECK_APPLY_STAGE2_ARGS();
+    return dual_apply_stage2_launch(N, d, h, cov_factor_ws, n_layers, layer_index, use_inverse, assembled, W0, W, dW_out, workspace,
+                                    info_dev, true, (hipStream_t)stream);
+}
+
+double* emcid_edit_dual_kt(void* workspace, int64_t N, int64_t d, int64_t h) { return dual_block(workspace, N, d, h, &DualWorkspace::off_K); }
+
+double* emcid_edit_dual_r(void* workspace, int64_t N, int64_t d, int64_t h) { return dual_block(workspace, N, d, h, &DualWorkspace::off_R); }
+
+double* emcid_edit_dual_rt(void* workspace, int64_t N, int64_t d, int64_t h) { return dual_block(workspace, N, d, h, &DualWorkspace::off_PT); }
 
 __global__ __launch_bounds__(256) void add_identity_f64_kernel(double* __restrict__ S, int n) {
     const int i = blockIdx.x * 256 + threadIdx.x;
diff --git a/emcid_amd/csrc/gemm_sp16.hip b/emcid_amd/csrc/gemm_sp16.hip
--- a/emcid_amd/csrc/gemm_sp16.hip
+++ b/emcid_amd/csrc/gemm_sp16.hip
@@ -714,18 +714,6 @@
     if constexpr (DBG == 2) {
         if (a.stamps != nullptr && threadIdx.x == 0) a.stamps[8 * (int64_t)blockIdx.x + 5] = (long long)__builtin_amdgcn_s_memrealtime();
     }
-}
-
-__device__ __forceinline__ void sp_split8(const v4f& a, const v4f& b, float s, v4u& hi, v4u& lo) {
-    v8h h, l;
-#pragma unroll
-    for (int e = 0; e < 8; ++e) {
-        const float t = (e < 4 ? a[e] : b[e - 4]) * s;
-        h[e] = (_Float16)t;
-        l[e] = (_Float16)(t - (float)h[e]);
-    }
-    hi = *reinterpret_cast<v4u*>(&h);
-    lo = *reinterpret_cast<v4u*>(&l);
 }
 
 __global__ __launch_bounds__(256) void split_rows_kernel(const float* __restrict__ X, int64_t ldx, int rows, int K,
diff --git a/emcid_amd/csrc/sp16.h b/emcid_amd/csrc/sp16.h
--- a/emcid_amd/csrc/sp16.h
+++ b/emcid_amd/csrc/sp16.h
@@ -26,4 +26,20 @@
     *reinterpret_cast<sp_v4h*>(dst + 16) = l;
 }
 
+typedef _Float16 sp_v8h __attribute__((ext_vector_type(8)));
+typedef float sp_v4f __attribute__((ext_vector_type(4)));
+typedef unsigned int sp_v4u __attribute__((ext_vector_type(4)));
+
+__device__ __forceinline__ void sp_split8(const sp_v4f& a, const sp_v4f& b, float s, sp_v4u& hi, sp_v4u& lo) {
+    sp_v8h h, l;
+#pragma unroll
+    for (int e = 0; e < 8; ++e) {
+        const float t = (e < 4 ? a[e] : b[e - 4]) * s;
+        h[e] = (_Float16)t;
+        l[e] = (_Float16)(t - (float)h[e]);
+    }
+    hi = *reinterpret_cast<sp_v4u*>(&h);
+    lo = *reinterpret_cast<sp_v4u*>(&l);
 }
+
+}
diff --git a/emcid_amd/csrc/spd_solve.h b/emcid_amd/csrc/spd_solve.h
--- a/emcid_amd/csrc/spd_solve.h
+++ b/emcid_amd/csrc/spd_solve.h
@@ -97,7 +97,7 @@
 };
 
 int solve_schur_rhs(const double* R, int64_t hp, int64_t h, int64_t Np, const double* LS, const double* invS, const double* XT,
-                    double* full_inv, double* RT, double* Y2, hipStream_t st);
+                    double* full_inv, double* RT, double* Y2, hipStream_t st, bool rt_filled = false);
 
 
 static __global__ __launch_bounds__(256) void copy2d_f64_kernel(const double* __restrict__ src, int64_t lds_, double* __restrict__ dst,
diff --git a/emcid_amd/hip.py b/emcid_amd/hip.py
--- a/emcid_amd/hip.py
+++ b/emcid_amd/hip.py
@@ -23,6 +23,8 @@
     "emcid_edit_dual_stage1_f64", "emcid_edit_dual_pt", "emcid_edit_dual_stage2_f64",
     "emcid_edit_dual_apply_stage1_f64", "emcid_edit_dual_yt", "emcid_edit_dual_apply_stage2_f64",
     "emcid_edit_dual_apply_assemble_f64",
+    "emcid_edit_dual_apply_stage1_rt_f64", "emcid_edit_dual_apply_stage2_rt_f64", "emcid_edit_keys_f64",
+    "emcid_edit_dual_kt", "emcid_edit_dual_r", "emcid_edit_dual_rt",
     "emcid_edit_dual_preserve_workspace_bytes", "emcid_edit_layer_dual_preserve_f64",
     "emcid_session_retain_workspace_bytes", "emcid_session_retain_f64", "emcid_session_step_norms_f64",
     "emcid_session_release_workspace_bytes", "emcid_session_release_f64",
@@ -86,6 +88,12 @@
         "emcid_edit_dual_yt": (p, [p, i64, i64, i64]),
         "emcid_edit_dual_apply_stage2_f64": (i32, [i64, i64, i64, p, i64, i64, i32, i32, p, p, p, p, i64, p, p]),
         "emcid_edit_dual_apply_assemble_f64": (i32, [i64, i64, i64, p, i64, p]),
+        "emcid_edit_dual_apply_stage1_rt_f64": (i32, [p, p, p, i64, i64, i64, f64, i32, f64, p, i64, i64, i64, i64, i32, p, i64, p]),
+        "emcid_edit_dual_apply_stage2_rt_f64": (i32, [i64, i64, i64, p, i64, i64, i32, i32, p, p, p, p, i64, p, p]),
+        "emcid_edit_keys_f64": (i32, [p, i64, p, p, i64, i64, i64, i64, f64, f64, p, p, p, p, i64, p]),
+        "emcid_edit_dual_kt": (p, [p, i64, i64, i64]),
+        "emcid_edit_dual_r": (p, [p, i64, i64, i64]),
+        "emcid_edit_dual_rt": (p, [p, i64, i64, i64]),
         "emcid_edit_dual_preserve_workspace_bytes": (i64, [i64, i64, i64, i64]),
         "emcid_edit_layer_dual_preserve_f64": (i32, [p, p, p, i64, i64, i64, f64, i32, f64, p, i64, i64, p, i64, p, i64, p, i64, i64,
                                                      p, p, p, p, p, i64, p, p]),
@@ -185,6 +193,7 @@
 
 
 
+FUSED_KEYS = os.environ.get("EMCID_FUSED_KEYS", "1") != "0"
 GRAM_SPLIT = os.environ.get("EMCID_GRAM_SPLIT", "1") != "0"
 _GRAM_WS = {}
 
@@ -984,6 +993,12 @@
         self.S = self.buf[off:off + self.Np * self.Np].view(self.Np, self.Np)
         off = (load().emcid_edit_dual_u(_ptr(self.buf), N, d, h) - self.buf.data_ptr()) // 8
         self.U = self.buf[off:off + hp * self.dp].view(hp, self.dp)[:h]
+        def block(fn, rows, cols):
+            o = (fn(_ptr(self.buf), N, d, h) - self.buf.data_ptr()) // 8
+            return self.buf[o:o + rows * cols].view(rows, cols)
+        self.Kt = block(load().emcid_edit_dual_kt, self.Np, self.dp)
+        self.R = block(load().emcid_edit_dual_r, self.Np, hp)
+        self.RT = block(load().emcid_edit_dual_rt, hp, self.Np)
 
 
 def edit_layer_dual(K, Zc, zs_t, factors: CovFactors, layer_index: int, edit_weight: float, layers_left: int,
@@ -1087,6 +1102,33 @@
     return {"dW": dW, "ws": ws}
 
 
+def edit_keys(act: torch.Tensor, lookup: torch.Tensor, seg: torch.Tensor, h: int, factors: CovFactors, edit_weight: float,
+              ws: DualWorkspace, lam: Optional[float] = None):
+    n_rows, d = act.shape
+    N = seg.numel() - 1
+    assert act.is_contiguous() and ws.key == (N, d, h)
+    K = torch.empty(N, d, dtype=torch.float32, device=act.device)
+    kp = torch.empty(N, d, dtype=torch.int32, device=act.device)
+    ks = torch.empty(N, dtype=torch.float32, device=act.device)
+    _check(load().emcid_edit_keys_f64(_ptr(act, torch.float32, "act"), n_rows, _ptr(lookup, torch.int64, "lookup"),
+                                      _ptr(seg, torch.int64, "seg"), lookup.numel(), N, d, h, float(edit_weight),
+                                      factors.lam_ratio(lam), _ptr(K), _ptr(kp), _ptr(ks), _ptr(ws.buf), ws.nbytes, _stream(act)),
+           "emcid_edit_keys_f64")
+    return K, SplitRows(kp, ks, K)
+
+
+def edit_dual_apply_stage1(K, Zc, zs_t, factors: CovFactors, layer_index: int, edit_weight: float, layers_left: int,
+                           ws: DualWorkspace, rt: bool, use_inverse: bool = True, lam: Optional[float] = None):
+    N, h = Zc.shape
+    d = factors.d
+    assert ws.key == (N, d, h) and (rt or K is not None)
+    name = "emcid_edit_dual_apply_stage1_rt_f64" if rt else "emcid_edit_dual_apply_stage1_f64"
+    _check(getattr(load(), name)(
+        _ptr(K, torch.float32, "K"), _ptr(Zc, torch.float32, "Zc"), _ptr(zs_t, torch.float32, "zs_t"), N, d, h,
+        float(edit_weight), int(layers_left), factors.lam_ratio(lam), _ptr(factors.buf), factors.n_layers, int(layer_index), 0, N,
+        int(bool(use_inverse)), _ptr(ws.buf), ws.nbytes, _stream(Zc)), name)
+
+
 def edit_layer_dual_apply(K, Zc, zs_t, factors: CovFactors, layer_index: int, edit_weight: float, layers_left: int,
                           W0, W, want_dw: bool = True, ws: Optional[DualWorkspace] = None,
                           use_inverse: Optional[bool] = None, on_factor_start=None, lam: Optional[float] = None):
@@ -1100,20 +1142,18 @@
     if ws is None or ws.key != (N, d, h):
         ws = DualWorkspace(N, d, h, K.device)
     lib = load()
-    _check(lib.emcid_edit_dual_apply_stage1_f64(
-        _ptr(K, torch.float32, "K"), _ptr(Zc, torch.float32, "Zc"), _ptr(zs_t, torch.float32, "zs_t"), N, d, h,
-        float(edit_weight), int(layers_left), factors.lam_ratio(lam), _ptr(factors.buf), factors.n_layers, int(layer_index), 0, N,
-        int(bool(use_inverse)), _ptr(ws.buf), ws.nbytes, _stream(K)), "emcid_edit_dual_apply_stage1_f64")
+    stage2 = "emcid_edit_dual_apply_stage2_rt_f64" if FUSED_KEYS else "emcid_edit_dual_apply_stage2_f64"
+    edit_dual_apply_stage1(K, Zc, zs_t, factors, layer_index, edit_weight, layers_left, ws, rt=FUSED_KEYS, use_inverse=use_inverse,
+                           lam=lam)
     dW = torch.empty(h, d, dtype=torch.float32, device=K.device) if want_dw else None
     if on_factor_start is not None:
         _check(lib.emcid_edit_dual_apply_assemble_f64(N, d, h, _ptr(ws.buf), ws.nbytes, _stream(K)),
                "emcid_edit_dual_apply_assemble_f64")
         on_factor_start()
-    _check(lib.emcid_edit_dual_apply_stage2_f64(N, d, h, _ptr(factors.buf), factors.n_layers, int(layer_index),
-                                                int(bool(use_inverse)), int(on_factor_start is not None),
-                                                _ptr(W0, torch.float32, "W0"), _ptr(W, torch.float32, "W"), _ptr(dW),
-                                                _ptr(ws.buf), ws.nbytes, _ptr(ws.info, torch.int32), _stream(K)),
-           "emcid_edit_dual_apply_stage2_f64")
+    _check(getattr(lib, stage2)(N, d, h, _ptr(factors.buf), factors.n_layers, int(layer_index),
+                                int(bool(use_inverse)), int(on_factor_start is not None),
+                                _ptr(W0, torch.float32, "W0"), _ptr(W, torch.float32, "W"), _ptr(dW),
+                                _ptr(ws.buf), ws.nbytes, _ptr(ws.info, torch.int32), _stream(K)), stage2)
     return {"dW": dW, "ws": ws}
 
 
diff --git a/include/emcid_hip.h b/include/emcid_hip.h
--- a/include/emcid_hip.h
+++ b/include/emcid_hip.h
@@ -160,6 +160,19 @@
 int emcid_edit_dual_apply_stage2_f64(int64_t N, int64_t d, int64_t h, const void* cov_factor_ws, int64_t n_layers,
                                      int64_t layer_index, int use_inverse, int assembled, const float* W0, float* W,
                                      float* dW_out, void* workspace, int64_t workspace_bytes, int* info_dev, void* stream);
+int emcid_edit_dual_apply_stage1_rt_f64(const float* K, const float* Zc, const float* zs_t, int64_t N, int64_t d, int64_t h,
+                                        double edit_weight, int layers_left, double lam_ratio, const void* cov_factor_ws,
+                                        int64_t n_layers, int64_t layer_index, int64_t n_lo, int64_t n_hi, int use_inverse,
+                                        void* workspace, int64_t workspace_bytes, void* stream);
+int emcid_edit_dual_apply_stage2_rt_f64(int64_t N, int64_t d, int64_t h, const void* cov_factor_ws, int64_t n_layers,
+                                        int64_t layer_index, int use_inverse, int assembled, const float* W0, float* W,
+                                        float* dW_out, void* workspace, int64_t workspace_bytes, int* info_dev, void* stream);
+int emcid_edit_keys_f64(const float* act, int64_t n_rows, const int64_t* lookup, const int64_t* seg, int64_t B, int64_t N, int64_t d,
+                        int64_t h, double edit_weight, double lam_ratio, float* K_out, void* k_planes, float* k_inv_scale,
+                        void* workspace, int64_t workspace_bytes, void* stream);
+double* emcid_edit_dual_kt(void* workspace, int64_t N, int64_t d, int64_t h);
+double* emcid_edit_dual_r(void* workspace, int64_t N, int64_t d, int64_t h);
+double* emcid_edit_dual_rt(void* workspace, int64_t N, int64_t d, int64_t h);
 int emcid_edit_dual_apply_assemble_f64(int64_t N, int64_t d, int64_t h, void* workspace, int64_t workspace_bytes, void* stream);
 
 int64_t emcid_edit_dual_preserve_workspace_bytes(int64_t N, int64_t d, int64_t h, int64_t capacity);
```
